# AgentMaker/PAPC

Hardware: AMD Instinct MI355X
Metric: point-clouds/sec (fwd+bwd) PointNet++SSG B=32 N=4096 (higher is better)
Workload: dtype f32

## Files before the change

### papc_amd/csrc/bn_ops.hip

```cpp
#include "common.h"

namespace papc {

template <int V> struct Vec;
template <> struct Vec<4> {
    float4 v;
    __device__ static Vec load(const float *p) { Vec r; r.v = *reinterpret_cast<const float4 *>(p); return r; }
    __device__ void store(float *p) const { *reinterpret_cast<float4 *>(p) = v; }
    __device__ float &operator[](int i) { return (&v.x)[i]; }
    __device__ float operator[](int i) const { return (&v.x)[i]; }
};
template <> struct Vec<1> {
    float v;
    __device__ static Vec load(const float *p) { Vec r; r.v = *p; return r; }
    __device__ void store(float *p) const { *p = v; }
    __device__ float &operator[](int) { return v; }
    __device__ float operator[](int) const { return v; }
};

template <int D>
__device__ __forceinline__ void sum_partial_rows_d(const float *__restrict__ part, int n_tiles, int C, int c, int tl, double &s1, double &s2)
{
    for (int t0 = tl; t0 < n_tiles; t0 += 64 * D) {
        float a[D], b[D];
#pragma unroll
        for (int j = 0; j < D; ++j) {
            const int t = t0 + 64 * j;
            const int64_t o = (int64_t)(t < n_tiles ? t : t0) * 2 * C + c;
            a[j] = part[o];
            b[j] = part[o + C];
        }
#pragma unroll
        for (int j = 0; j < D; ++j) {
            if (t0 + 64 * j < n_tiles) { s1 += (double)a[j]; s2 += (double)b[j]; }
        }
    }
}
__device__ __forceinline__ void sum_partial_rows(const float *__restrict__ part, int n_tiles, int C, int c, int tl, double &s1, double &s2)
{
    if (n_tiles > 512) sum_partial_rows_d<16>(part, n_tiles, C, c, tl, s1, s2);
    else sum_partial_rows_d<8>(part, n_tiles, C, c, tl, s1, s2);
}

__device__ __forceinline__ double lane_get(double v, int l)
{
    const int lo = __builtin_amdgcn_readlane(__double2loint(v), l), hi = __builtin_amdgcn_readlane(__double2hiint(v), l);
    return __hiloint2double(hi, lo);
}
__device__ __forceinline__ void fold_part_lanes(double &s1, double &s2)
{
    s1 += __shfl_xor(s1, 1); s2 += __shfl_xor(s2, 1);
    s1 += __shfl_xor(s1, 2); s2 += __shfl_xor(s2, 2);
    double t1 = 0.0, t2 = 0.0;
#pragma unroll
    for (int w = 0; w < 16; ++w) { t1 += lane_get(s1, 4 * w); t2 += lane_get(s2, 4 * w); }
    s1 = t1; s2 = t2;
}

__device__ __forceinline__ void bn_finalize_channel(const int c, const float *__restrict__ part, int n_tiles, int64_t M, int C,
                                                    const float *__restrict__ gamma, const float *__restrict__ beta,
                                                    float eps, float momentum, float *mean, float *invstd, float *scale,
                                                    float *shift, float *rmean, float *rvar)
{
    const int tl = threadIdx.x;
    const float gam = gamma ? gamma[c] : 1.f, bet = beta ? beta[c] : 0.f;
    const float rm0 = rmean ? rmean[c] : 0.f, rv0 = rvar ? rvar[c] : 0.f;
    double s1 = 0.0, s2 = 0.0;
    sum_partial_rows(part, n_tiles, C, c, tl, s1, s2);
    fold_part_lanes(s1, s2);
    if (tl == 0) {
        const double mu = s1 / (double)M;
        double var = s2 / (double)M - mu * mu;
        if (var < 0.0) var = 0.0;
        const double is = 1.0 / sqrt(var + (double)eps);
        const double sc = (double)gam * is;
        mean[c] = (float)mu;
        invstd[c] = (float)is;
        scale[c] = (float)sc;
        shift[c] = (float)((double)bet - mu * sc);
        if (rmean) rmean[c] = momentum * rm0 + (1.f - momentum) * (float)mu;
        if (rvar) rvar[c] = momentum * rv0 + (1.f - momentum) * (float)var;
    }
}
__global__ __launch_bounds__(64) void bn_finalize_kernel(const float *__restrict__ part, int n_tiles, int64_t M, int C,
                                                        const float *__restrict__ gamma, const float *__restrict__ beta,
                                                        float eps, float momentum, float *mean, float *invstd, float *scale,
                                                        float *shift, float *rmean, float *rvar)
{
    bn_finalize_channel(blockIdx.x, part, n_tiles, M, C, gamma, beta, eps, momentum, mean, invstd, scale, shift, rmean, rvar);
}
constexpr int BN_CLEAR_PER_LANE = 16, BN_CLEAR_PER_WG = 64 * BN_CLEAR_PER_LANE;
__global__ __launch_bounds__(64) void bn_finalize_clear_kernel(const float *__restrict__ part, int n_tiles, int64_t M, int C,
                                                              const float *__restrict__ gamma, const float *__restrict__ beta,
                                                              float eps, float momentum, float *mean, float *invstd, float *scale,
                                                              float *shift, float *rmean, float *rvar, uint4 *__restrict__ clr, int64_t n16)
{
    if ((int)blockIdx.x >= C) {
        const int64_t i0 = (int64_t)((int)blockIdx.x - C) * BN_CLEAR_PER_WG + threadIdx.x;
#pragma unroll
        for (int q = 0; q < BN_CLEAR_PER_LANE; ++q) {
            const int64_t i = i0 + q * 64;
            if (i < n16) clr[i] = make_uint4(0u, 0u, 0u, 0u);
        }
        return;
    }
    bn_finalize_channel(blockIdx.x, part, n_tiles, M, C, gamma, beta, eps, momentum, mean, invstd, scale, shift, rmean, rvar);
}

template <int V>
__global__ __launch_bounds__(256) void bn_relu_max_kernel(const float *__restrict__ y, const float *__restrict__ scale,
                                                          const float *__restrict__ shift, int64_t G, int K, int C,
                                                          float *__restrict__ out, int32_t *__restrict__ argmax)
{
    const int CV = C / V;
    const int64_t total = G * CV;
    for (int64_t e = (int64_t)blockIdx.x * blockDim.x + threadIdx.x; e < total; e += (int64_t)gridDim.x * blockDim.x) {
        const int64_t g = e / CV;
        const int c = (int)(e - g * CV) * V;
        const Vec<V> sc = Vec<V>::load(scale + c), sh = Vec<V>::load(shift + c);
        Vec<V> best;
        int bi[V];
#pragma unroll
        for (int i = 0; i < V; ++i) { best[i] = -1.0f; bi[i] = 0; }
        const float *yp = y + (g * K) * (int64_t)C + c;
        for (int k = 0; k < K; ++k) {
            const Vec<V> v = Vec<V>::load(yp + (int64_t)k * C);
#pragma unroll
            for (int i = 0; i < V; ++i) {
                const float z = relu_np(fmaf(sc[i], v[i], sh[i]));
                if (z > best[i] || z != z) { best[i] = z; bi[i] = k; }
            }
        }
        best.store(out + g * C + c);
        if (argmax) {
#pragma unroll
            for (int i = 0; i < V; ++i) argmax[g * C + c + i] = bi[i];
        }
    }
}

__global__ __launch_bounds__(256) void bn_select_max_kernel(float *__restrict__ gmax, const float *__restrict__ gmin,
                                                            const int32_t *__restrict__ amax, const int32_t *__restrict__ amin,
                                                            const float *__restrict__ scale, const float *__restrict__ shift,
                                                            int64_t total, int C, float *__restrict__ out, int32_t *__restrict__ argmax)
{
    for (int64_t e = (int64_t)blockIdx.x * blockDim.x + threadIdx.x; e < total; e += (int64_t)gridDim.x * blockDim.x) {
        const int c = (int)(e % C);
        const float sc = scale[c], sh = shift[c];
        const bool up = sc >= 0.f;
        const float sel = up ? gmax[e] : gmin[e];
        out[e] = relu_np(fmaf(sc, sel, sh));
        gmax[e] = sel;
        if (argmax) argmax[e] = up ? amax[e] : amin[e];
    }
}

template <int V>
__global__ __launch_bounds__(256) void bn_relu_kernel(const float *__restrict__ y, const float *__restrict__ scale,
                                                      const float *__restrict__ shift, int64_t M, int C, float *__restrict__ z)
{
    const int CV = C / V;
    const int64_t total = M * CV;
    for (int64_t e = (int64_t)blockIdx.x * blockDim.x + threadIdx.x; e < total; e += (int64_t)gridDim.x * blockDim.x) {
        const int c = (int)(e % CV) * V;
        const Vec<V> sc = Vec<V>::load(scale + c), sh = Vec<V>::load(shift + c);
        Vec<V> v = Vec<V>::load(y + e * V);
#pragma unroll
        for (int i = 0; i < V; ++i) v[i] = fmaxf(fmaf(sc[i], v[i], sh[i]), 0.f);
        v.store(z + e * V);
    }
}

template <int V, bool MAXMODE>
__global__ __launch_bounds__(256) void bn_bwd_reduce_kernel(const float *__restrict__ dz, const float *__restrict__ gout,
                                                            const int32_t *__restrict__ argmax, int K,
                                                            const float *__restrict__ y, const float *__restrict__ mean,
                                                            const float *__restrict__ invstd, const float *__restrict__ scale,
                                                            const float *__restrict__ shift, int64_t M, int C,
                                                            float *__restrict__ part, float *__restrict__ psel_out = nullptr)
{
    __shared__ float red[2][256 * 4];
    const int CV = C / V;
    const int CG = CV < 256 ? CV : 256;
    const int RL = 256 / CG;
    const int cgi = threadIdx.x % CG, rl = threadIdx.x / CG;
    const int64_t units = MAXMODE ? M / K : M;
    const int64_t per = (units + gridDim.x - 1) / gridDim.x;
    const int64_t u0 = (int64_t)blockIdx.x * per, u1 = min(units, u0 + per);

    for (int cb = 0; cb < CV; cb += CG) {
        const int cg = cb + cgi;
        Vec<V> a1, a2;
#pragma unroll
        for (int i = 0; i < V; ++i) { a1[i] = 0.f; a2[i] = 0.f; }
        if (cg < CV && rl < RL) {
            const int c = cg * V;
            const Vec<V> sc = Vec<V>::load(scale + c), sh = Vec<V>::load(shift + c);
            const Vec<V> mu = Vec<V>::load(mean + c), is = Vec<V>::load(invstd + c);
            for (int64_t u = u0 + rl; u < u1; u += RL) {
                if (MAXMODE) {
                    Vec<V> g = Vec<V>::load(gout + u * C + c);
                    Vec<V> ys;
                    if (dz) {
                        ys = Vec<V>::load(dz + u * C + c);
                    } else {
#pragma unroll
                        for (int i = 0; i < V; ++i) ys[i] = y[(u * K + argmax[u * C + c + i]) * (int64_t)C + c + i];
                    }
#pragma unroll
                    for (int i = 0; i < V; ++i) {
                        const float yv = ys[i];
                        const float z = fmaf(sc[i], yv, sh[i]);
                        const float p = z > 0.f ? g[i] : 0.f;
                        a1[i] += p;
                        a2[i] = fmaf(p, (yv - mu[i]) * is[i], a2[i]);
                        g[i] = sc[i] * p;
                    }
                    if (psel_out) g.store(psel_out + u * C + c);
                } else {
                    const Vec<V> d = Vec<V>::load(dz + u * C + c);
                    const Vec<V> yv = Vec<V>::load(y + u * C + c);
#pragma unroll
                    for (int i = 0; i < V; ++i) {
                        const float z = fmaf(sc[i], yv[i], sh[i]);
                        const float p = z > 0.f ? d[i] : 0.f;
                        a1[i] += p;
                        a2[i] = fmaf(p, (yv[i] - mu[i]) * is[i], a2[i]);
                    }
                }
            }
        }
#pragma unroll
        for (int i = 0; i < V; ++i) { red[0][threadIdx.x * V + i] = a1[i]; red[1][threadIdx.x * V + i] = a2[i]; }
        __syncthreads();
        for (int t = threadIdx.x; t < CG * V; t += 256) {
            const int c = cb * V + t;
            if (c < C) {
                const int g = t / V, i = t - g * V;
                float s1 = 0.f, s2 = 0.f;
                for (int r = 0; r < RL; ++r) { s1 += red[0][(r * CG + g) * V + i]; s2 += red[1][(r * CG + g) * V + i]; }
                part[((int64_t)blockIdx.x * 2 + 0) * C + c] = s1;
                part[((int64_t)blockIdx.x * 2 + 1) * C + c] = s2;
            }
        }
        __syncthreads();
    }
}

__global__ __launch_bounds__(64) void bn_bwd_finalize_kernel(const float *__restrict__ part, int n_tiles, int64_t M, int C,
                                                            float *dgamma, float *dbeta, float *c1, float *c2, int accumulate)
{
    const int c = blockIdx.x, tl = threadIdx.x;
    double s1 = 0.0, s2 = 0.0;
    sum_partial_rows(part, n_tiles, C, c, tl, s1, s2);
    fold_part_lanes(s1, s2);
    if (tl == 0) {
        if (dbeta) dbeta[c] = (accumulate & 1) ? dbeta[c] + (float)s1 : (float)s1;
        if (dgamma) dgamma[c] = (accumulate & 1) ? dgamma[c] + (float)s2 : (float)s2;
        const bool eval_bn = (accumulate & 2) != 0;
        c1[c] = eval_bn ? 0.f : (float)(s1 / (double)M);
        c2[c] = eval_bn ? 0.f : (float)(s2 / (double)M);
    }
}

__global__ void bn_eval_consts_kernel(const float *__restrict__ rmean, const float *__restrict__ rvar, const float *__restrict__ gamma,
                                      const float *__restrict__ beta, float eps, int C, float *mean, float *invstd, float *scale, float *shift)
{
    const int c = blockIdx.x * blockDim.x + threadIdx.x;
    if (c >= C) return;
    const double mu = (double)rmean[c];
    const double is = 1.0 / sqrt((double)rvar[c] + (double)eps);
    const double sc = (gamma ? (double)gamma[c] : 1.0) * is;
    mean[c] = (float)mu;
    invstd[c] = (float)is;
    scale[c] = (float)sc;
    shift[c] = (float)((beta ? (double)beta[c] : 0.0) - mu * sc);
}

__global__ __launch_bounds__(256) void group_max_bwd_kernel(const float *__restrict__ gout, const int32_t *__restrict__ argmax, int64_t G,
                                                            int K, int C, float *__restrict__ dx)
{
    const int64_t total = G * K * (int64_t)C;
    for (int64_t e = (int64_t)blockIdx.x * blockDim.x + threadIdx.x; e < total; e += (int64_t)gridDim.x * blockDim.x) {
        const int c = (int)(e % C);
        const int64_t m = e / C;
        const int64_t g = m / K;
        const int k = (int)(m - g * K);
        dx[e] = (argmax[g * C + c] == k) ? gout[g * C + c] : 0.f;
    }
}

template <bool ZERO>
__global__ __launch_bounds__(256) void adam_kernel(float *__restrict__ p, float *__restrict__ g, float *__restrict__ m,
                                                   float *__restrict__ v, int64_t n, float lr, float b1, float b2, float omb1, float omb2,
                                                   float eps, float wd, float bc1, float bc2, float gscale)
{
    for (int64_t i = (int64_t)blockIdx.x * blockDim.x + threadIdx.x; i < n; i += (int64_t)gridDim.x * blockDim.x) {
        float gi = g[i] * gscale + wd * p[i];
        const float mi = b1 * m[i] + omb1 * gi;
        const float vi = b2 * v[i] + omb2 * gi * gi;
        m[i] = mi; v[i] = vi;
        p[i] -= lr * (mi / bc1) / (sqrtf(vi / bc2) + eps);
        if (ZERO) g[i] = 0.f;
    }
}

template <bool ZERO, bool TICK, int V>
__global__ __launch_bounds__(256) void adam_dev_kernel(float *__restrict__ p, float *__restrict__ g, float *__restrict__ m,
                                                       float *__restrict__ v, int64_t n, float lr, double beta1, double beta2,
                                                       float eps, float wd, int64_t *__restrict__ step_dev, float gscale)
{
    __shared__ float s_bc[2];
    __shared__ int64_t s_t;
    const int64_t nv = n / V, stride = (int64_t)gridDim.x * blockDim.x, i0 = (int64_t)blockIdx.x * blockDim.x + threadIdx.x;
    Vec<V> gq, pq, mq, vq;
    if (i0 < nv) { gq = Vec<V>::load(g + i0 * V); pq = Vec<V>::load(p + i0 * V); mq = Vec<V>::load(m + i0 * V); vq = Vec<V>::load(v + i0 * V); }
    if (threadIdx.x == 0) {
        const int64_t ti = step_dev[0] + (TICK ? 1 : 0);
        const double t = (double)ti;
        s_t = ti;
        s_bc[0] = (float)(1.0 - pow(beta1, t));
        s_bc[1] = (float)(1.0 - pow(beta2, t));
    }
    __syncthreads();
    const float bc1 = s_bc[0], bc2 = s_bc[1];
    const float b1 = (float)beta1, b2 = (float)beta2, omb1 = (float)(1.0 - beta1), omb2 = (float)(1.0 - beta2);
    for (int64_t i = i0; i < nv; i += stride) {
        if (i != i0) { gq = Vec<V>::load(g + i * V); pq = Vec<V>::load(p + i * V); mq = Vec<V>::load(m + i * V); vq = Vec<V>::load(v + i * V); }
#pragma unroll
        for (int e = 0; e < V; ++e) {
            const float gi = gq[e] * gscale + wd * pq[e];
            const float mi = b1 * mq[e] + omb1 * gi;
            const float vi = b2 * vq[e] + omb2 * gi * gi;
            mq[e] = mi; vq[e] = vi;
            pq[e] -= lr * (mi / bc1) / (sqrtf(vi / bc2) + eps);
            gq[e] = 0.f;
        }
        mq.store(m + i * V); vq.store(v + i * V); pq.store(p + i * V);
        if (ZERO) gq.store(g + i * V);
    }
    if (TICK) {
        __syncthreads();
        if (threadIdx.x == 0) {
            const unsigned long long done = atomicAdd(reinterpret_cast<unsigned long long *>(step_dev + 1), 1ull);
            if (done == (unsigned long long)gridDim.x - 1ull) {
                step_dev[0] = s_t;
                __hip_atomic_store(reinterpret_cast<unsigned long long *>(step_dev + 1), 0ull, __ATOMIC_RELAXED, __HIP_MEMORY_SCOPE_AGENT);
            }
        }
    }
}
__global__ void adam_tick_kernel(int64_t *step_dev) { step_dev[0] += 1; }

__global__ void flag_set_kernel(unsigned *flag, unsigned value, int64_t *counter)
{
    if (counter) counter[0] += 1;
    __hip_atomic_fetch_add(flag, value, __ATOMIC_RELEASE, __HIP_MEMORY_SCOPE_AGENT);
}
__global__ void flag_wait_kernel(unsigned *flag, long long max_spins, int widx)
{
    if (threadIdx.x != 0) return;
    const unsigned want = flag[widx] + 1u;
    long long n = 0;
    while ((int)(__hip_atomic_load(flag, __ATOMIC_ACQUIRE, __HIP_MEMORY_SCOPE_AGENT) - want) < 0) {
        if (n >= max_spins) { __hip_atomic_fetch_add(flag + 2, 1u, __ATOMIC_RELAXED, __HIP_MEMORY_SCOPE_AGENT); break; }
        __builtin_amdgcn_s_sleep(32);
        ++n;
    }
    flag[widx] = want;
}

__global__ __launch_bounds__(256) void fill_kernel(float *__restrict__ p, int64_t n, float v)
{
    const int64_t n4 = n >> 2;
    float4 *p4 = reinterpret_cast<float4 *>(p);
    const float4 v4 = make_float4(v, v, v, v);
    for (int64_t i = (int64_t)blockIdx.x * blockDim.x + threadIdx.x; i < n4; i += (int64_t)gridDim.x * blockDim.x) p4[i] = v4;
    if (blockIdx.x == 0 && threadIdx.x < (n & 3)) p[(n4 << 2) + threadIdx.x] = v;
}

__global__ __launch_bounds__(256) void copy2d_kernel(const float *__restrict__ src, int64_t src_ld, float *__restrict__ dst, int64_t dst_ld,
                                                     int rows, int cols, int transpose)
{
    const int64_t total = (int64_t)rows * cols;
    for (int64_t e = (int64_t)blockIdx.x * blockDim.x + threadIdx.x; e < total; e += (int64_t)gridDim.x * blockDim.x) {
        int r, c;
        if (transpose) { c = (int)(e / rows); r = (int)(e - (int64_t)c * rows); dst[(int64_t)c * dst_ld + r] = src[(int64_t)r * src_ld + c]; }
        else { r = (int)(e / cols); c = (int)(e - (int64_t)r * cols); dst[(int64_t)r * dst_ld + c] = src[(int64_t)r * src_ld + c]; }
    }
}

struct CopyJobs {
    const float *src[8];
    float *dst[8];
    int B[8], R[8], C[8];
    int64_t sb[8], sr[8], sc[8], db[8], dr[8], dc[8];
};

__global__ __launch_bounds__(256) void copy_strided_batch_kernel(CopyJobs j)
{
    __shared__ float tile[32][33];
    const int q = blockIdx.y;
    const int R = j.R[q], C = j.C[q];
    const int tr = (R + 31) >> 5, tc = (C + 31) >> 5;
    const int64_t ntiles = (int64_t)j.B[q] * tr * tc;
    const float *src = j.src[q];
    float *dst = j.dst[q];
    const int64_t sb = j.sb[q], sr = j.sr[q], sc = j.sc[q], db = j.db[q], dr = j.dr[q], dc = j.dc[q];
    const bool src_along_c = sc == 1 || sr != 1, dst_along_c = dc == 1 || dr != 1;
    const int tx = threadIdx.x & 31, ty = threadIdx.x >> 5;
    for (int64_t t = blockIdx.x; t < ntiles; t += gridDim.x) {
        const int b = (int)(t / (tr * tc));
        const int rem = (int)(t - (int64_t)b * tr * tc);
        const int r0 = (rem / tc) * 32, c0 = (rem % tc) * 32;
#pragma unroll
// ... 474 lines not shown
```

### papc_amd/csrc/capi.hip

```cpp
#include <stdarg.h>
#include <string.h>

#include <mutex>
#include <vector>

#include "common.h"

#define GEMM_PARTS_DEFAULT 768

namespace papc {

static thread_local char g_err[512] = "";

void set_error(const char *fmt, ...)
{
    va_list ap;
    va_start(ap, fmt);
    vsnprintf(g_err, sizeof(g_err), fmt, ap);
    va_end(ap);
}

int check_launch(const char *what)
{
    hipError_t e = hipGetLastError();
    if (e != hipSuccess) {
        set_error("%s: %s", what, hipGetErrorString(e));
        return PAPC_E_LAUNCH;
    }
    return PAPC_OK;
}

struct KnobDef { const char *name; int def, lo, hi; };
static const KnobDef g_knob_defs[KNOB_COUNT] = {
    {"PAPC_LG_PARTS", 2048, 1, 8192},
    {"PAPC_DW_F32", 0, 0, 1},
    {"PAPC_DW_DBG", 0, 0, 1},
    {"PAPC_DW_XYZ", 1, 0, 1},
    {"PAPC_PARTS", GEMM_PARTS_DEFAULT, 1, 1024},
    {"PAPC_GEMM_F32", 0, 0, 1},
    {"PAPC_GEMM_WAVES", 0, 0, 8},
    {"PAPC_MAXCAT_WAVES", 8, 4, 8},
    {"PAPC_GEMM_WS", 0, 0, 3},
    {"PAPC_GEMM_OCC", 0, 0, 1},
    {"PAPC_GEMM_DBG", 0, 0, 1},
    {"PAPC_GEMM_KB", 0, 0, 2},
    {"PAPC_GEMM_MINWG", 192, 1, 4096},
    {"PAPC_GEMM_TL", 0, 0, 1},
    {"PAPC_FPS_THREADS", 0, 0, 1024},
    {"PAPC_FPS_THREADS_SMALL", 0, 0, 1024},
    {"PAPC_STREAM", 1, 0, 1},
    {"PAPC_STREAM_MINTILES", 2048, 1, 1 << 30},
    {"PAPC_STREAM_CK", 0, 0, 8},
    {"PAPC_STREAM_ASM", 1, 0, 1},
    {"PAPC_PFN_MFMA", 1, 0, 1},
    {"PAPC_DW_RS64", 1, 0, 1},
    {"PAPC_DW_ROWS", 1, 0, 1},
    {"PAPC_DW_ROWS_BLOCKS", 4, 1, 16},
    {"PAPC_DW_ROWSX", 1, 0, 1},
    {"PAPC_PG_DBG", 0, 0, 15},
    {"PAPC_PG_NB", 0, 0, 2},
    {"PAPC_PG_NS", 0, 0, 3},
    {"PAPC_STREAM_MAXCAT", 1, 0, 1},
    {"PAPC_MAX_NOSTORE", 1, 0, 1},
    {"PAPC_PFN_FUSED_TAILS", 1, 0, 1},
    {"PAPC_STREAM_NW12", 1, 0, 1},
    {"PAPC_LG_LISTS", 1, 0, 1},
    {"PAPC_FOLD_WAVES", 16, 8, 16},
    {"PAPC_LGL_VARIANT", 0, 0, 3},
    {"PAPC_LG_PP", 1, 0, 1},
    {"PAPC_PG_GROUP", 1, 0, 1},
    {"PAPC_PG_PIPE", 1, 0, 1},
    {"PAPC_SEG_EPI", 1, 0, 1},
};
static int g_knobs[KNOB_COUNT];
static int knob_parse(int id, const char *e)
{
    const KnobDef &d = g_knob_defs[id];
    if (!e || !*e) return d.def;
    const int v = atoi(e);
    return (v < d.lo || v > d.hi) ? d.def : v;
}
static const bool g_knobs_loaded = [] {
    for (int i = 0; i < KNOB_COUNT; ++i) g_knobs[i] = knob_parse(i, getenv(g_knob_defs[i].name));
    return true;
}();
int knob(int id) { return g_knobs[id]; }

struct ProfState {
    std::mutex mu;
    unsigned mask = 0;
    std::vector<std::pair<hipEvent_t, hipEvent_t>> pending[PAPC_K_COUNT];
    std::vector<hipEvent_t> pool;
    double total_ms[PAPC_K_COUNT] = {0};
    int64_t launches[PAPC_K_COUNT] = {0};
};
static ProfState g_prof;

static hipEvent_t prof_get_event()
{
    if (!g_prof.pool.empty()) {
        hipEvent_t e = g_prof.pool.back();
        g_prof.pool.pop_back();
        return e;
    }
    hipEvent_t e;
    if (hipEventCreate(&e) != hipSuccess) return nullptr;
    return e;
}

ProfScope::ProfScope(int k, hipStream_t s) : kernel(k), stream(s), on(false), e0(nullptr)
{
    if (!(g_prof.mask & (1u << k))) return;
    std::lock_guard<std::mutex> lk(g_prof.mu);
    e0 = prof_get_event();
    if (!e0) return;
    on = hipEventRecord(e0, stream) == hipSuccess;
}

ProfScope::~ProfScope()
{
    if (!on) return;
    std::lock_guard<std::mutex> lk(g_prof.mu);
    hipEvent_t e1 = prof_get_event();
    if (!e1) return;
    if (hipEventRecord(e1, stream) == hipSuccess) g_prof.pending[kernel].push_back({e0, e1});
}

static void prof_drain(int k)
{
    for (auto &pr : g_prof.pending[k]) {
        float ms = 0.f;
        if (hipEventSynchronize(pr.second) == hipSuccess && hipEventElapsedTime(&ms, pr.first, pr.second) == hipSuccess) {
            g_prof.total_ms[k] += ms;
            g_prof.launches[k] += 1;
        }
        g_prof.pool.push_back(pr.first);
        g_prof.pool.push_back(pr.second);
    }
    g_prof.pending[k].clear();
}

}

extern "C" {

int papc_version(void) { return 600;  }

int papc_abi_version(void) { return PAPC_ABI_VERSION; }

int64_t papc_abi_sizeof(const char *struct_name)
{
    if (!struct_name) return -1;
#define PAPC_SIZEOF(T) if (strcmp(struct_name, #T) == 0) return (int64_t)sizeof(T);
    PAPC_SIZEOF(papc_group_src)
    PAPC_SIZEOF(papc_point_lists)
    PAPC_SIZEOF(papc_group_max)
    PAPC_SIZEOF(papc_bwd_dy)
    PAPC_SIZEOF(papc_scatter_dst)
    PAPC_SIZEOF(papc_bwd_red)
    PAPC_SIZEOF(papc_reduce_job)
    PAPC_SIZEOF(papc_fold_job)
    PAPC_SIZEOF(papc_fold_list)
    PAPC_SIZEOF(papc_sa_desc)
    PAPC_SIZEOF(papc_sa_layer)
    PAPC_SIZEOF(papc_compact_src)
    PAPC_SIZEOF(papc_sa_io)
    PAPC_SIZEOF(papc_sa_plan)
    PAPC_SIZEOF(papc_sa_grads)
    PAPC_SIZEOF(papc_pfn_desc)
    PAPC_SIZEOF(papc_pfn_io)
    PAPC_SIZEOF(papc_det_loss_desc)
    PAPC_SIZEOF(papc_det_loss_io)
    PAPC_SIZEOF(papc_det_post_desc)
    PAPC_SIZEOF(papc_det_post_io)
    PAPC_SIZEOF(papc_head_fc_layer)
    PAPC_SIZEOF(papc_head_bwd_job)
    PAPC_SIZEOF(papc_pg_wjob)
    PAPC_SIZEOF(papc_pg_prep)
    PAPC_SIZEOF(papc_pg_gemm)
    PAPC_SIZEOF(papc_pg_fold_job)
    PAPC_SIZEOF(papc_copy_job)
#undef PAPC_SIZEOF
    return -1;
}

const char *papc_last_error_string(void) { return papc::g_err; }

int papc_knob_set(const char *name, int value)
{
    PAPC_REQUIRE(name, PAPC_E_INVALID, "papc_knob_set: null name");
    for (int i = 0; i < papc::KNOB_COUNT; ++i)
        if (!strcmp(name, papc::g_knob_defs[i].name)) {
            PAPC_REQUIRE(value >= papc::g_knob_defs[i].lo && value <= papc::g_knob_defs[i].hi, PAPC_E_INVALID,
                         "papc_knob_set: %s = %d outside [%d, %d]", name, value, papc::g_knob_defs[i].lo, papc::g_knob_defs[i].hi);
            papc::g_knobs[i] = value;
            return PAPC_OK;
        }
    papc::set_error("papc_knob_set: unknown knob %s", name);
    return PAPC_E_INVALID;
}

int papc_knob_get(const char *name, int *value)
{
    PAPC_REQUIRE(name && value, PAPC_E_INVALID, "papc_knob_get: null argument");
    for (int i = 0; i < papc::KNOB_COUNT; ++i)
        if (!strcmp(name, papc::g_knob_defs[i].name)) { *value = papc::g_knobs[i]; return PAPC_OK; }
    papc::set_error("papc_knob_get: unknown knob %s", name);
    return PAPC_E_INVALID;
}

int papc_prof_enable(unsigned mask)
{
    std::lock_guard<std::mutex> lk(papc::g_prof.mu);
    papc::g_prof.mask = mask;
    return PAPC_OK;
}

int papc_prof_reset(void)
{
    std::lock_guard<std::mutex> lk(papc::g_prof.mu);
    for (int k = 0; k < PAPC_K_COUNT; ++k) {
        papc::prof_drain(k);
        papc::g_prof.total_ms[k] = 0;
        papc::g_prof.launches[k] = 0;
    }
// ... 15 lines not shown
```

### papc_amd/csrc/common.h

```cpp
#pragma once
#include <hip/hip_runtime.h>
#include <stdint.h>
#include <stdio.h>
#include <stdlib.h>
#include <string.h>
#include <algorithm>

#include "papc_hip.h"

namespace papc {

void set_error(const char *fmt, ...);
int check_launch(const char *what);

#define PAPC_REQUIRE(cond, code, ...)      \
    do {                                   \
        if (!(cond)) {                     \
            papc::set_error(__VA_ARGS__);  \
            return (code);                 \
        }                                  \
    } while (0)

enum Knob {
    KNOB_LG_PARTS, KNOB_DW_F32, KNOB_DW_DBG, KNOB_DW_XYZ, KNOB_PARTS, KNOB_GEMM_F32, KNOB_GEMM_WAVES, KNOB_MAXCAT_WAVES,
    KNOB_GEMM_WS, KNOB_GEMM_OCC, KNOB_GEMM_DBG, KNOB_GEMM_KB, KNOB_GEMM_MINWG, KNOB_GEMM_TL, KNOB_FPS_THREADS,
    KNOB_FPS_THREADS_SMALL, KNOB_STREAM, KNOB_STREAM_MINTILES, KNOB_STREAM_CK, KNOB_STREAM_ASM, KNOB_PFN_MFMA, KNOB_DW_RS64, KNOB_DW_ROWS, KNOB_DW_ROWS_BLOCKS, KNOB_DW_ROWSX, KNOB_PG_DBG, KNOB_PG_NB, KNOB_PG_NS, KNOB_STREAM_MAXCAT, KNOB_MAX_NOSTORE, KNOB_PFN_FUSED_TAILS, KNOB_STREAM_NW12, KNOB_LG_LISTS, KNOB_FOLD_WAVES, KNOB_LGL_VARIANT, KNOB_LG_PP, KNOB_PG_GROUP, KNOB_PG_PIPE, KNOB_SEG_EPI, KNOB_COUNT
};
int knob(int id);

struct ProfScope {
    int kernel;
    hipStream_t stream;
    bool on;
    hipEvent_t e0;
    ProfScope(int kernel, hipStream_t stream);
    ~ProfScope();
};

static inline hipStream_t as_stream(papc_stream_t s) { return reinterpret_cast<hipStream_t>(s); }

static inline int64_t cdiv(int64_t a, int64_t b) { return (a + b - 1) / b; }
static inline bool aligned16(const void *p) { return (reinterpret_cast<uintptr_t>(p) & 15) == 0; }

#define PAPC_DPP(v, ctrl, rmask) __builtin_amdgcn_update_dpp((int)(v), (int)(v), (ctrl), (rmask), 0xF, false)

__device__ __forceinline__ float wave_sum_f32_to_lane63(float v)
{
    float t;
    t = __int_as_float(PAPC_DPP(__float_as_int(v), 0xB1, 0xF));  v += t;
    t = __int_as_float(PAPC_DPP(__float_as_int(v), 0x4E, 0xF));  v += t;
    t = __int_as_float(PAPC_DPP(__float_as_int(v), 0x124, 0xF)); v += t;
    t = __int_as_float(PAPC_DPP(__float_as_int(v), 0x128, 0xF)); v += t;
    t = __int_as_float(__builtin_amdgcn_update_dpp(0, __float_as_int(v), 0x142, 0xA, 0xF, false)); v += t;
    t = __int_as_float(__builtin_amdgcn_update_dpp(0, __float_as_int(v), 0x143, 0xC, 0xF, false)); v += t;
    return v;
}

__device__ __forceinline__ float half_sum_f32(float v)
{
    float t;
    t = __int_as_float(PAPC_DPP(__float_as_int(v), 0xB1, 0xF));  v += t;
    t = __int_as_float(PAPC_DPP(__float_as_int(v), 0x4E, 0xF));  v += t;
    t = __int_as_float(PAPC_DPP(__float_as_int(v), 0x124, 0xF)); v += t;
    t = __int_as_float(PAPC_DPP(__float_as_int(v), 0x128, 0xF)); v += t;
    t = __int_as_float(__builtin_amdgcn_update_dpp(0, __float_as_int(v), 0x142, 0xA, 0xF, false)); v += t;
    return v;
}

__device__ __forceinline__ float readlane63_f32(float v)
{
    return __int_as_float(__builtin_amdgcn_readlane(__float_as_int(v), 63));
}


#define PAPC_DPPF(v, ctrl, rmask) __int_as_float(__builtin_amdgcn_update_dpp(__float_as_int(v), __float_as_int(v), (ctrl), (rmask), 0xF, false))
#define PAPC_DPPU(v, ctrl, rmask) ((unsigned)__builtin_amdgcn_update_dpp((int)(v), (int)(v), (ctrl), (rmask), 0xF, false))

__device__ __forceinline__ float row_max_f32(float v)
{
    v = fmaxf(v, PAPC_DPPF(v, 0xB1, 0xF));
    v = fmaxf(v, PAPC_DPPF(v, 0x4E, 0xF));
    v = fmaxf(v, PAPC_DPPF(v, 0x124, 0xF));
    v = fmaxf(v, PAPC_DPPF(v, 0x128, 0xF));
    return v;
}
__device__ __forceinline__ unsigned row_min_u32(unsigned v)
{
    unsigned t;
    t = PAPC_DPPU(v, 0xB1, 0xF);  v = t < v ? t : v;
    t = PAPC_DPPU(v, 0x4E, 0xF);  v = t < v ? t : v;
    t = PAPC_DPPU(v, 0x124, 0xF); v = t < v ? t : v;
    t = PAPC_DPPU(v, 0x128, 0xF); v = t < v ? t : v;
    return v;
}
__device__ __forceinline__ float wave_max_f32_to_lane63(float v)
{
    v = row_max_f32(v);
    v = fmaxf(v, PAPC_DPPF(v, 0x142, 0xA));
    v = fmaxf(v, PAPC_DPPF(v, 0x143, 0xC));
    return v;
}
__device__ __forceinline__ unsigned wave_min_u32_to_lane63(unsigned v)
{
    unsigned t;
    v = row_min_u32(v);
    t = PAPC_DPPU(v, 0x142, 0xA); v = t < v ? t : v;
    t = PAPC_DPPU(v, 0x143, 0xC); v = t < v ? t : v;
    return v;
}
#define PAPC_DPP_STEP(op, v, ctrl) asm volatile("s_nop 1\n\t" op " %0, %0, %0 " ctrl : "+v"(v))
__device__ __forceinline__ unsigned row_max_u32_fused(unsigned v)
{
    PAPC_DPP_STEP("v_max_u32_dpp", v, "quad_perm:[1,0,3,2] row_mask:0xf bank_mask:0xf");
    PAPC_DPP_STEP("v_max_u32_dpp", v, "quad_perm:[2,3,0,1] row_mask:0xf bank_mask:0xf");
    PAPC_DPP_STEP("v_max_u32_dpp", v, "row_ror:4 row_mask:0xf bank_mask:0xf");
    PAPC_DPP_STEP("v_max_u32_dpp", v, "row_ror:8 row_mask:0xf bank_mask:0xf");
    return v;
}
__device__ __forceinline__ unsigned row_min_u32_fused(unsigned v)
{
    PAPC_DPP_STEP("v_min_u32_dpp", v, "quad_perm:[1,0,3,2] row_mask:0xf bank_mask:0xf");
    PAPC_DPP_STEP("v_min_u32_dpp", v, "quad_perm:[2,3,0,1] row_mask:0xf bank_mask:0xf");
    PAPC_DPP_STEP("v_min_u32_dpp", v, "row_ror:4 row_mask:0xf bank_mask:0xf");
    PAPC_DPP_STEP("v_min_u32_dpp", v, "row_ror:8 row_mask:0xf bank_mask:0xf");
    return v;
}
__device__ __forceinline__ unsigned wave_max_u32_fused_to_lane63(unsigned v)
{
    v = row_max_u32_fused(v);
    PAPC_DPP_STEP("v_max_u32_dpp", v, "row_bcast:15 row_mask:0xa bank_mask:0xf");
    PAPC_DPP_STEP("v_max_u32_dpp", v, "row_bcast:31 row_mask:0xc bank_mask:0xf");
    asm volatile("s_nop 1" ::"v"(v));
    return v;
}
__device__ __forceinline__ unsigned wave_min_u32_fused_to_lane63(unsigned v)
{
    v = row_min_u32_fused(v);
    PAPC_DPP_STEP("v_min_u32_dpp", v, "row_bcast:15 row_mask:0xa bank_mask:0xf");
    PAPC_DPP_STEP("v_min_u32_dpp", v, "row_bcast:31 row_mask:0xc bank_mask:0xf");
    asm volatile("s_nop 1" ::"v"(v));
    return v;
}
__device__ __forceinline__ unsigned readlane63_u32(unsigned v) { return (unsigned)__builtin_amdgcn_readlane((int)v, 63); }
__device__ __forceinline__ float readlane0_f32(float v) { return __int_as_float(__builtin_amdgcn_readlane(__float_as_int(v), 0)); }
__device__ __forceinline__ unsigned readlane0_u32(unsigned v) { return (unsigned)__builtin_amdgcn_readlane((int)v, 0); }

__device__ __forceinline__ void lds_barrier()
{
    asm volatile("s_waitcnt lgkmcnt(0)\n\ts_barrier" ::: "memory");
}

__device__ __forceinline__ float relu_np(float t) { return !(t <= 0.f) ? t : 0.f; }
__device__ __forceinline__ int lane_id() { return (int)(threadIdx.x & 63); }

}
```

### papc_amd/csrc/mlp_dw.hip

```cpp
#include <type_traits>
#include "mlp_loaders.h"

namespace papc {

template <int I, int N, class F>
__device__ __forceinline__ void dw_sfor(F &&f)
{
    if constexpr (I < N) {
        f(std::integral_constant<int, I>{});
        dw_sfor<I + 1, N>(f);
    }
}

void fill_dy(DySrc &d, const papc_bwd_dy *s);
int check_dy(const papc_bwd_dy *dy, int64_t M, int C, bool *vec, const char *who);
int fill_asrc(ASrc &a, int a_mode, const float *x, int64_t ldx, const papc_group_src *grp, const float *sc,
              const float *sh, int Cin, const char *who);

struct DwArgs {
    ASrc x;
    ASrc dy;
    int64_t M; int Cin; int Cout; int rows_per_chunk;
    float *dw_partial;
    float *db_partial;
    int64_t part_ld;
    int xmap;
    int TOp, TIp;
    int RS;
    unsigned long long *dbg;
};

constexpr int DW_T = 128;
constexpr int DW_TI_WIDE = 160;
constexpr int DW_STAGE_FLOATS = 9216;

template <int XMODE, int DYMODE, bool VEC, int WO, int WI, int NTO, int NTI, int NSX>
__global__ __launch_bounds__(256, 2) void dw_kernel(DwArgs p)
{
    static_assert(WO * WI == 4, "4 waves");
    __shared__ __attribute__((aligned(16))) float smem[2 * DW_STAGE_FLOATS + DW_T];
    float *dbred = smem + 2 * DW_STAGE_FLOATS;

    const int tid = threadIdx.x, lane = tid & 63, wave = tid >> 6;
    const int hi = lane >> 5, l31 = lane & 31;
    const int wo = wave / WI, wi = wave % WI;
    const int o0 = blockIdx.y * DW_T, i0 = blockIdx.z * (NSX > 4 ? DW_TI_WIDE : DW_T);
    const int TOp = p.TOp, TIp = p.TIp, RS = p.RS;
    const int nto = min(TOp / 32, (p.Cout - o0 + 31) / 32);
    const int nti = min(TIp / 32, (p.Cin - i0 + 31) / 32);
    const int cgy = TOp / 4, cgx = TIp / 4;
    const int nsy = (RS * cgy + 255) / 256, nsx = (RS * cgx + 255) / 256;
    int yr[4], xr[NSX], xk[NSX];
    const int kqy = (tid % cgy) * 4;
#pragma unroll
    for (int i = 0; i < 4; ++i) yr[i] = (tid + 256 * (i < nsy ? i : nsy - 1)) / cgy;
#pragma unroll
    for (int i = 0; i < NSX; ++i) {
        const int s = tid + 256 * (i < nsx ? i : nsx - 1);
        xr[i] = s / cgx;
        xk[i] = (s - xr[i] * cgx) * 4;
    }
    const int kqx = xk[0];
    const bool use_jpre = (XMODE == A_GROUP) && p.x.g.idx != nullptr;

    floatx16 acc[NTO][NTI];
#pragma unroll
    for (int a = 0; a < NTO; ++a)
#pragma unroll
        for (int b = 0; b < NTI; ++b)
#pragma unroll
            for (int r = 0; r < 16; ++r) acc[a][b][r] = 0.f;
    int toff[NTO], tiff[NTI];
    bool tok_o[NTO], tok_i[NTI];
#pragma unroll
    for (int a = 0; a < NTO; ++a) { const int to = wo * NTO + a; tok_o[a] = to < nto; toff[a] = (tok_o[a] ? to : 0) * 32; }
#pragma unroll
    for (int b = 0; b < NTI; ++b) { const int ti = wi * NTI + b; tok_i[b] = ti < nti; tiff[b] = (tok_i[b] ? ti : 0) * 32; }

    const KConst kcy = make_kconst<DYMODE, VEC>(p.dy, o0 + kqy, p.Cout);
    const KConst kcx = make_kconst<XMODE, VEC>(p.x, i0 + kqx, p.Cin);
    float4 dbs = make_float4(0.f, 0.f, 0.f, 0.f);

    const int64_t mbeg = (int64_t)blockIdx.x * p.rows_per_chunk;
    const int64_t mend = min(p.M, mbeg + p.rows_per_chunk);

    RowCtx rowy[4], rowx[NSX];
    Raw3 rawy[4], rawx[NSX];
    int jpre[NSX];
#pragma unroll
    for (int i = 0; i < NSX; ++i) jpre[i] = -2;

    auto prefetch_j = [&](int64_t m0) {
        if (use_jpre) {
#pragma unroll
            for (int i = 0; i < NSX; ++i) {
                const int64_t m = m0 + xr[i];
                jpre[i] = p.x.g.idx[m < p.M ? m : 0];
            }
        }
    };
    auto fetch = [&](int64_t m0) {
#pragma unroll
        for (int i = 0; i < 4; ++i) {
            rowy[i] = make_row<DYMODE>(p.dy, m0 + yr[i], mend);
            rawy[i] = fetch_a4<DYMODE, VEC>(p.dy, rowy[i], o0 + kqy, p.Cout);
        }
#pragma unroll
        for (int i = 0; i < NSX; ++i) {
            rowx[i] = make_row<XMODE>(p.x, m0 + xr[i], mend, use_jpre ? jpre[i] : -2);
            rawx[i] = fetch_a4<XMODE, VEC>(p.x, rowx[i], i0 + xk[i], p.Cin);
        }
    };
    auto finish = [&](float *Ys, float *Xs) {
#pragma unroll
        for (int i = 0; i < 4; ++i) {
            const float4 vy = finish_a4<DYMODE, VEC>(p.dy, rowy[i], o0 + kqy, p.Cout, kcy, rawy[i]);
            if (i < nsy) { dbs.x += vy.x; dbs.y += vy.y; dbs.z += vy.z; dbs.w += vy.w; }
            *reinterpret_cast<float4 *>(&Ys[yr[i] * TOp + kqy]) = vy;
        }
#pragma unroll
        for (int i = 0; i < NSX; ++i) {
            const float4 vx = finish_a4<XMODE, VEC>(p.x, rowx[i], i0 + xk[i], p.Cin, kcx, rawx[i]);
            *reinterpret_cast<float4 *>(&Xs[xr[i] * TIp + xk[i]]) = vx;
        }
    };

    bool have = mbeg < mend;
    if (have) {
        prefetch_j(mbeg);
        fetch(mbeg);
        prefetch_j(mbeg + RS);
        finish(smem, smem + RS * TOp);
    }
    __syncthreads();
    int buf = 0;
    int64_t m0 = mbeg;
    while (have) {
        const int64_t mn = m0 + RS;
        const bool have_next = mn < mend;
        if (have_next) {
            fetch(mn);
            prefetch_j(mn + RS);
        }
        {
            const float *Ys = smem + buf * DW_STAGE_FLOATS + hi * TOp + l31;
            const float *Xs = smem + buf * DW_STAGE_FLOATS + RS * TOp + hi * TIp + l31;
            const int nks = RS / 2;
            float a0[NTO], b0[NTI], a1[NTO], b1[NTI];
#pragma unroll
            for (int a = 0; a < NTO; ++a) a0[a] = Ys[toff[a]];
#pragma unroll
            for (int b = 0; b < NTI; ++b) b0[b] = Xs[tiff[b]];
            for (int ks = 0; ks < nks; ks += 2) {
                const float *y1 = Ys + (2 * ks + 2) * TOp, *x1 = Xs + (2 * ks + 2) * TIp;
#pragma unroll
                for (int a = 0; a < NTO; ++a) a1[a] = y1[toff[a]];
#pragma unroll
                for (int b = 0; b < NTI; ++b) b1[b] = x1[tiff[b]];
#pragma unroll
                for (int a = 0; a < NTO; ++a)
#pragma unroll
                    for (int b = 0; b < NTI; ++b) acc[a][b] = __builtin_amdgcn_mfma_f32_32x32x2f32(a0[a], b0[b], acc[a][b], 0, 0, 0);
                const int k2 = (ks + 2 < nks) ? ks + 2 : ks;
                const float *y2 = Ys + (2 * k2) * TOp, *x2 = Xs + (2 * k2) * TIp;
#pragma unroll
                for (int a = 0; a < NTO; ++a) a0[a] = y2[toff[a]];
#pragma unroll
                for (int b = 0; b < NTI; ++b) b0[b] = x2[tiff[b]];
#pragma unroll
                for (int a = 0; a < NTO; ++a)
#pragma unroll
                    for (int b = 0; b < NTI; ++b) acc[a][b] = __builtin_amdgcn_mfma_f32_32x32x2f32(a1[a], b1[b], acc[a][b], 0, 0, 0);
            }
        }
        if (have_next) {
            float *Ys = smem + (buf ^ 1) * DW_STAGE_FLOATS;
            finish(Ys, Ys + RS * TOp);
        }
        lds_barrier();
        buf ^= 1;
        m0 = mn;
        have = have_next;
// ... 360 lines not shown
    for (int a = 0; a < NTO; ++a) {
        const int c = o0 + 32 * a + l31;
        ksc[a] = d.scale[c]; ksh[a] = d.shift[c]; kmu[a] = d.mean[c];
        kA[a] = ksc[a] * d.c1[c];
        kB[a] = ksc[a] * d.c2[c] * d.invstd[c];
    }
#pragma unroll
    for (int b = 0; b < NTI; ++b) {
        if (XYZ) { xs[b] = 0.f; xh[b] = 0.f; }
        else { xs[b] = p.x.sc[i0 + 32 * b + l31]; xh[b] = p.x.sh[i0 + 32 * b + l31]; }
    }
    float4 wfk[NTI];
#pragma unroll
    for (int b = 0; b < NTI; ++b) wfk[b] = XYZ ? ld4(p.x.sc + 4 * (i0 + 32 * b + l31)) : make_float4(0.f, 0.f, 0.f, 0.f);

    floatx16 acc[NTO][NTI];
#pragma unroll
    for (int a = 0; a < NTO; ++a)
#pragma unroll
        for (int b = 0; b < NTI; ++b)
#pragma unroll
            for (int r = 0; r < 16; ++r) acc[a][b][r] = 0.f;

    struct Raw { float y[NTO][8], z[NTO][8], x[XYZ ? 3 : NTI][8]; int am[NTO]; };
    auto ldg = [](const float *base, uint32_t byte_off) { return *reinterpret_cast<const float *>(reinterpret_cast<const char *>(base) + byte_off); };
    auto ldgi = [](const int *base, uint32_t byte_off) { return *reinterpret_cast<const int *>(reinterpret_cast<const char *>(base) + byte_off); };
    const uint32_t ystride = (uint32_t)Cout * 4u, xstride = (uint32_t)(XYZ ? 4 : ldx) * 4u;
    const uint32_t oy_lane = (uint32_t)((mbeg + 8 * hi) * Cout + o0 + l31) * 4u;
    const uint32_t ox_lane = XYZ ? (uint32_t)((mbeg + 8 * hi) * 4) * 4u : (uint32_t)((mbeg + 8 * hi) * ldx + i0 + l31) * 4u;
    auto fetch = [&](int kb, Raw &w) {
        const uint32_t oy = oy_lane + (uint32_t)kb * 16u * ystride, ox = ox_lane + (uint32_t)kb * 16u * xstride;
#pragma unroll
        for (int j = 0; j < 8; ++j) {
#pragma unroll
            for (int a = 0; a < NTO; ++a) {
                w.y[a][j] = ldg(d.y, oy + (uint32_t)j * ystride + 128u * a);
                if (DYMODE == A_DY_DENSE) w.z[a][j] = ldg(d.dz, oy + (uint32_t)j * ystride + 128u * a);
            }
            if (XYZ) {
                w.x[0][j] = ldg(p.x.x, ox + (uint32_t)j * 16u); w.x[1][j] = ldg(p.x.x, ox + (uint32_t)j * 16u + 4u); w.x[2][j] = ldg(p.x.x, ox + (uint32_t)j * 16u + 8u);
            } else {
#pragma unroll
                for (int b = 0; b < NTI; ++b) w.x[b][j] = ldg(p.x.x, ox + (uint32_t)j * xstride + 128u * b);
            }
        }
        if (DYMODE == A_DY_MAX) {
            const uint32_t g = fdiv((uint32_t)mbeg + 16u * (uint32_t)kb, d.divK);
            const uint32_t og = (g * (uint32_t)Cout + (uint32_t)(o0 + l31)) * 4u;
#pragma unroll
            for (int a = 0; a < NTO; ++a) {
                w.z[a][0] = ldg(d.gout, og + 128u * a);
                w.am[a] = ldgi(d.argmax, og + 128u * a);
            }
        }
    };
    auto compute = [&](int kb, const Raw &w) {
        int kin0 = 0;
        if (DYMODE == A_DY_MAX) {
            const uint32_t b0 = (uint32_t)mbeg + 16u * (uint32_t)kb;
            kin0 = (int)(b0 - fdiv(b0, d.divK) * (uint32_t)d.K) + 8 * hi;
        }
        bf16x8 pa[NTO][3], pb[NTI][3];
#pragma unroll
        for (int a = 0; a < NTO; ++a) {
            float v[8];
#pragma unroll
            for (int j = 0; j < 8; ++j) {
                const float y = w.y[a][j];
                float dz;
                if (DYMODE == A_DY_DENSE) dz = w.z[a][j];
                else dz = (w.am[a] == kin0 + j) ? w.z[a][0] : 0.f;
                const float z = fmaf(ksc[a], y, ksh[a]);
                const float pp = z > 0.f ? dz : 0.f;
                v[j] = fmaf(ksc[a], pp, -fmaf(kB[a], y - kmu[a], kA[a]));
            }
            split8(v, pa[a]);
        }
#pragma unroll
        for (int b = 0; b < NTI; ++b) {
            float v[8];
#pragma unroll
            for (int j = 0; j < 8; ++j) {
                if (XYZ) v[j] = fmaxf(fmaf(wfk[b].z, w.x[2][j], fmaf(wfk[b].y, w.x[1][j], fmaf(wfk[b].x, w.x[0][j], wfk[b].w))), 0.f);
                else v[j] = fmaxf(fmaf(xs[b], w.x[b][j], xh[b]), 0.f);
            }
            split8(v, pb[b]);
        }
#pragma unroll
        for (int t = 0; t < 6; ++t)
#pragma unroll
            for (int a = 0; a < NTO; ++a)
#pragma unroll
                for (int b = 0; b < NTI; ++b)
                    acc[a][b] = __builtin_amdgcn_mfma_f32_32x32x16_bf16(pa[a][BF16X3_PA[t]], pb[b][BF16X3_PB[t]], acc[a][b], 0, 0, 0);
    };

    constexpr int PF = (DYMODE == A_DY_MAX && !XYZ) ? 3 : 2;
    const int nb = (n_kb - wave + 7) >> 3;
    if (nb > 0) {
        const int last = wave + 8 * (nb - 1);
        Raw rr[PF];
#pragma unroll
        for (int i = 0; i < PF - 1; ++i) fetch(min(wave + 8 * i, last), rr[i]);
        const int n_main = nb - nb % PF;
        for (int j0 = 0; j0 < n_main; j0 += PF) {
#pragma unroll
            for (int i = 0; i < PF; ++i) {
                const int kb = wave + 8 * (j0 + i);
                fetch(min(kb + 8 * (PF - 1), last), rr[(i + PF - 1) % PF]);
                __builtin_amdgcn_sched_barrier(0);
                compute(kb, rr[i]);
                __builtin_amdgcn_sched_barrier(0);
            }
        }
#pragma unroll
        for (int i = 0; i < PF - 1; ++i)
            if (n_main + i < nb) compute(wave + 8 * (n_main + i), rr[i]);
    }

#pragma unroll
    for (int half = 4; half >= 1; half >>= 1) {
        if (wave >= half && wave < 2 * half) {
#pragma unroll
            for (int a = 0; a < NTO; ++a)
#pragma unroll
                for (int b = 0; b < NTI; ++b)
#pragma unroll
                    for (int r = 0; r < 16; ++r) slab[wave - half][(a * NTI + b) * 16 + r][lane] = acc[a][b][r];
        }
        __syncthreads();
        if (wave < half) {
#pragma unroll
            for (int a = 0; a < NTO; ++a)
#pragma unroll
                for (int b = 0; b < NTI; ++b)
#pragma unroll
                    for (int r = 0; r < 16; ++r) acc[a][b][r] += slab[wave][(a * NTI + b) * 16 + r][lane];
        }
        __syncthreads();
    }
    if (wave == 0) {
        float *out = p.dw_partial + (int64_t)blockIdx.x * p.part_ld;
#pragma unroll
        for (int a = 0; a < NTO; ++a)
#pragma unroll
            for (int b = 0; b < NTI; ++b)
#pragma unroll
                for (int r = 0; r < 16; ++r) {
                    const int co = o0 + 32 * a + (r & 3) + 8 * (r >> 2) + 4 * hi;
                    out[(int64_t)co * p.Cin + i0 + 32 * b + l31] = acc[a][b][r];
                }
    }
    if (p.db_partial && blockIdx.z == 0 && tid < 64) p.db_partial[(int64_t)blockIdx.x * p.part_ld + o0 + tid] = 0.f;
}

template <int DYMODE, int NW, bool CP = false, bool RG = false>
__global__ __launch_bounds__(64 * NW, 2) void dw_rowsx_kernel(DwArgs p)
{
    static_assert(!(CP && RG), "ragged widths: padded stacks only");
    constexpr int NTI = 4, CI = 128, CHS = 48, PLB = CI * CHS, STG = 3 * PLB;
    constexpr int CB = 32 * NW;
    constexpr int RPT = 32 / NW;
    constexpr int NX4 = RPT / 4;
    __shared__ __attribute__((aligned(16))) char xs_lds[2 * STG];
    const int tid = threadIdx.x, lane = tid & 63, wave = tid >> 6;
    const int hi = lane >> 5, l31 = lane & 31;
    const int co = RG ? min((int)blockIdx.y * CB + wave * 32 + l31, p.Cout - 1) : blockIdx.y * CB + wave * 32 + l31;
    const DySrc &d = p.dy.d;
    const int i0 = RG ? (int)blockIdx.z * CI : 0;
    const uint32_t LDX = RG ? (uint32_t)p.x.ldx : (uint32_t)CI;
    int64_t rows_all = p.M, rpc = p.rows_per_chunk;
    if constexpr (CP) {
        rows_all = __builtin_amdgcn_readfirstlane(*d.rows_dev);
        rpc = (((rows_all + gridDim.x - 1) / gridDim.x) + 15) & ~(int64_t)15;
    }
    const int64_t mbeg = (int64_t)blockIdx.x * rpc;
    const int64_t mend = min(rows_all, mbeg + rpc);
    const int n_kb = mbeg < mend ? (int)((mend - mbeg) >> 4) : 0;
    const int Cout = p.Cout;

    const float ksc = d.scale[co], ksh = d.shift[co], kmu = d.mean[co];
    const float kA = ksc * d.c1[co], kB = ksc * d.c2[co] * d.invstd[co];
    const int xc = tid & 127, xq = tid >> 7;
    const int xg = RG ? min(i0 + xc, p.Cin - 1) : xc;
    const float xsc = p.x.sc[xg], xsh = p.x.sh[xg];

    floatx16 acc[NTI];
#pragma unroll
    for (int b = 0; b < NTI; ++b)
#pragma unroll
        for (int r = 0; r < 16; ++r) acc[b][r] = 0.f;

    struct Raw { float y[8], z[8]; int am; float4 w0, w1; int g; };
    struct RawX { float x[RPT]; };
    auto ldg = [](const float *base, uint32_t byte_off) { return *reinterpret_cast<const float *>(reinterpret_cast<const char *>(base) + byte_off); };
    auto ldgi = [](const int *base, uint32_t byte_off) { return *reinterpret_cast<const int *>(reinterpret_cast<const char *>(base) + byte_off); };
    const uint32_t ystride = (uint32_t)Cout * 4u;
    const uint32_t oy_lane = (uint32_t)((mbeg + 8 * hi) * Cout + co) * 4u;
    const uint32_t ox_lane = (uint32_t)((mbeg + RPT * xq) * LDX + xg) * 4u;
    const uint32_t ow_lane = (uint32_t)(mbeg + 8 * hi) * 4u;
    const uint32_t og_lane = (uint32_t)(((mbeg >> 3) + hi)) * 4u;
    auto fetch_g = [&](int kb, Raw &w) {
        if constexpr (CP && DYMODE == A_DY_MAX) w.g = ldgi(d.seg_grp, og_lane + (uint32_t)kb * 8u);
    };
    auto fetch = [&](int kb, Raw &w) {
        const uint32_t o0 = oy_lane + (uint32_t)kb * 16u * ystride;
#pragma unroll
        for (int j = 0; j < 8; ++j) {
            w.y[j] = ldg(d.y, o0 + (uint32_t)j * ystride);
            if (DYMODE == A_DY_DENSE) w.z[j] = ldg(d.dz, o0 + (uint32_t)j * ystride);
        }
        if (DYMODE == A_DY_MAX) {
            uint32_t g;
            if constexpr (CP) g = (uint32_t)w.g;
            else g = fdiv((uint32_t)mbeg + 16u * (uint32_t)kb, d.divK);
            const uint32_t og = (g * (uint32_t)Cout + (uint32_t)co) * 4u;
            w.z[0] = ldg(d.gout, og);
            w.am = ldgi(d.argmax, og);
        }
        if constexpr (CP) {
            const char *wb = reinterpret_cast<const char *>(d.wrow) + ow_lane + (uint32_t)kb * 64u;
            w.w0 = *reinterpret_cast<const float4 *>(wb);
            w.w1 = *reinterpret_cast<const float4 *>(wb + 16);
        }
    };
    auto wof = [](const Raw &w, int j) -> float {
        const float a[8] = {w.w0.x, w.w0.y, w.w0.z, w.w0.w, w.w1.x, w.w1.y, w.w1.z, w.w1.w};
        return a[j];
    };
    auto fetch_x = [&](int kb, RawX &w) {
        const uint32_t o0 = ox_lane + (uint32_t)kb * (16u * LDX * 4u);
#pragma unroll
        for (int j = 0; j < RPT; ++j) w.x[j] = ldg(p.x.x, o0 + (uint32_t)j * (LDX * 4u));
    };
    auto stage_x = [&](int kb, const RawX &w, char *stg) {
        (void)kb;
#pragma unroll
        for (int h = 0; h < NX4; ++h) {
            float4 v;
            v.x = fmaxf(fmaf(xsc, w.x[4 * h + 0], xsh), 0.f); v.y = fmaxf(fmaf(xsc, w.x[4 * h + 1], xsh), 0.f);
            v.z = fmaxf(fmaf(xsc, w.x[4 * h + 2], xsh), 0.f); v.w = fmaxf(fmaf(xsc, w.x[4 * h + 3], xsh), 0.f);
            uint2 q0, q1, q2;
            split3(v, q0, q1, q2);
            char *dst = stg + xc * CHS + xq * (2 * RPT) + 8 * h;
            *reinterpret_cast<uint2 *>(dst) = q0;
            *reinterpret_cast<uint2 *>(dst + PLB) = q1;
            *reinterpret_cast<uint2 *>(dst + 2 * PLB) = q2;
        }
    };
    auto prep = [&](int kb, const Raw &w, bf16x8 (&pa)[3]) {
        int kin0 = 0;
        if (DYMODE == A_DY_MAX) {
            const uint32_t b0 = (uint32_t)mbeg + 16u * (uint32_t)kb;
            kin0 = CP ? (int)b0 + 8 * hi : (int)(b0 - fdiv(b0, d.divK) * (uint32_t)d.K) + 8 * hi;
        }
        float v[8];
#pragma unroll
        for (int j = 0; j < 8; ++j) {
            const float y = w.y[j];
            float dz;
            if (DYMODE == A_DY_DENSE) dz = w.z[j];
            else dz = (w.am == kin0 + j) ? w.z[0] : 0.f;
            const float z = fmaf(ksc, y, ksh);
            const float pp = z > 0.f ? dz : 0.f;
            if constexpr (CP) v[j] = fmaf(-wof(w, j), fmaf(kB, y - kmu, kA), ksc * pp);
            else v[j] = fmaf(ksc, pp, -fmaf(kB, y - kmu, kA));
        }
        split8(v, pa);
    };
    auto mma = [&](const bf16x8 (&pa)[3], const char *stg) {
        bf16x8 pb[NTI][3];
#pragma unroll
        for (int b = 0; b < NTI; ++b)
#pragma unroll
            for (int pl = 0; pl < 3; ++pl)
                pb[b][pl] = *reinterpret_cast<const bf16x8 *>(stg + pl * PLB + (32 * b + l31) * CHS + hi * 16);
#pragma unroll
        for (int t = 0; t < 6; ++t)
#pragma unroll
            for (int b = 0; b < NTI; ++b)
                acc[b] = __builtin_amdgcn_mfma_f32_32x32x16_bf16(pa[BF16X3_PA[t]], pb[b][BF16X3_PB[t]], acc[b], 0, 0, 0);
    };

    auto weave = [&](const bf16x8 (&pc)[3], const char *stg, int kbn, const Raw &w, bf16x8 (&pn)[3], const RawX &wx, char *stgn) {
        bf16x8 pb[NTI][3];
#pragma unroll
        for (int pl = 0; pl < 3; ++pl)
#pragma unroll
            for (int b = 0; b < NTI; ++b)
                pb[b][pl] = *reinterpret_cast<const bf16x8 *>(stg + pl * PLB + (32 * b + l31) * CHS + hi * 16);
        int kin0 = 0;
        if (DYMODE == A_DY_MAX) {
            const uint32_t b0 = (uint32_t)mbeg + 16u * (uint32_t)kbn;
            kin0 = CP ? (int)b0 + 8 * hi : (int)(b0 - fdiv(b0, d.divK) * (uint32_t)d.K) + 8 * hi;
        }
        float v[8];
        float4 ra, rb, rx;
        uint2 a0, a1, a2, b0, b1, b2, q0, q1, q2;
        auto pin = [](float &x) { asm volatile("" : "+v"(x)); };
        auto pin4 = [&](float4 &r) { pin(r.x); pin(r.y); pin(r.z); pin(r.w); };
        auto pinu = [](uint2 &u) { asm volatile("" : "+v"(u.x), "+v"(u.y)); };
        dw_sfor<0, 24>([&](auto g_) {
            constexpr int g = decltype(g_)::value, t = g / NTI, bb = g % NTI;
            acc[bb] = __builtin_amdgcn_mfma_f32_32x32x16_bf16(pc[BF16X3_PA[t]], pb[bb][BF16X3_PB[t]], acc[bb], 0, 0, 0);
            __builtin_amdgcn_sched_barrier(0);
            if constexpr (g < 8) {
                const float y = w.y[g];
                float dz;
                if (DYMODE == A_DY_DENSE) dz = w.z[g];
                else dz = (w.am == kin0 + g) ? w.z[0] : 0.f;
                const float z = fmaf(ksc, y, ksh);
                const float pp = z > 0.f ? dz : 0.f;
                if constexpr (CP) v[g] = fmaf(-wof(w, g), fmaf(kB, y - kmu, kA), ksc * pp);
                else v[g] = fmaf(ksc, pp, -fmaf(kB, y - kmu, kA));
                pin(v[g]);
            } else if constexpr (g == 8) { ra = make_float4(v[0], v[1], v[2], v[3]); split_level(ra, a0); pin4(ra); pinu(a0); }
            else if constexpr (g == 9) { split_level(ra, a1); pin4(ra); pinu(a1); }
            else if constexpr (g == 10) {
                a2.x = pack_bf16x2(ra.x, ra.y); a2.y = pack_bf16x2(ra.z, ra.w); rb = make_float4(v[4], v[5], v[6], v[7]); split_level(rb, b0);
                pinu(a2); pin4(rb); pinu(b0);
            } else if constexpr (g == 11) { split_level(rb, b1); pin4(rb); pinu(b1); }
            else if constexpr (g == 12) {
                b2.x = pack_bf16x2(rb.x, rb.y); b2.y = pack_bf16x2(rb.z, rb.w);
                pinu(b2);
                pn[0] = __builtin_bit_cast(bf16x8, make_uint4(a0.x, a0.y, b0.x, b0.y));
                pn[1] = __builtin_bit_cast(bf16x8, make_uint4(a1.x, a1.y, b1.x, b1.y));
                pn[2] = __builtin_bit_cast(bf16x8, make_uint4(a2.x, a2.y, b2.x, b2.y));
            } else if constexpr (g >= 13 && g < 13 + 4 * NX4) {
                constexpr int h = (g - 13) / 4, step = (g - 13) % 4;
                if constexpr (step == 0) {
                    rx.x = fmaxf(fmaf(xsc, wx.x[4 * h + 0], xsh), 0.f); rx.y = fmaxf(fmaf(xsc, wx.x[4 * h + 1], xsh), 0.f);
                    rx.z = fmaxf(fmaf(xsc, wx.x[4 * h + 2], xsh), 0.f); rx.w = fmaxf(fmaf(xsc, wx.x[4 * h + 3], xsh), 0.f);
                    pin4(rx);
                } else if constexpr (step == 1) { split_level(rx, q0); pin4(rx); pinu(q0); }
                else if constexpr (step == 2) { split_level(rx, q1); pin4(rx); pinu(q1); }
                else {
                    q2.x = pack_bf16x2(rx.x, rx.y); q2.y = pack_bf16x2(rx.z, rx.w);
                    char *dst = stgn + xc * CHS + xq * (2 * RPT) + 8 * h;
                    *reinterpret_cast<uint2 *>(dst) = q0;
                    *reinterpret_cast<uint2 *>(dst + PLB) = q1;
                    *reinterpret_cast<uint2 *>(dst + 2 * PLB) = q2;
                }
            }
            __builtin_amdgcn_sched_barrier(0);
        });
    };

    constexpr int PF = 3;
    Raw dr[PF];
    RawX xr[PF];
    bf16x8 pa[PF][3];
    const int last = n_kb - 1;
    if (n_kb > 0) {
#pragma unroll
        for (int i = 0; i < PF; ++i) fetch_g(min(i, last), dr[i]);
#pragma unroll
        for (int i = 0; i < PF - 1; ++i) { fetch(min(i, last), dr[i]); fetch_x(min(i, last), xr[i]); }
        stage_x(0, xr[0], xs_lds);
        prep(0, dr[0], pa[0]);
        lds_barrier();
    }
    const int n_main = n_kb - n_kb % PF;
    for (int kb0 = 0; kb0 < n_main; kb0 += PF) {
#pragma unroll
        for (int i = 0; i < PF; ++i) {
            const int kb = kb0 + i;
            constexpr int NXT = PF - 1;
            if constexpr (CP && DYMODE == A_DY_MAX) {
                const int gnew = ldgi(d.seg_grp, og_lane + (uint32_t)min(kb + PF, last) * 8u);
                fetch(min(kb + NXT, last), dr[(i + NXT) % PF]);
                dr[i].g = gnew;
            } else
            fetch(min(kb + NXT, last), dr[(i + NXT) % PF]);
            fetch_x(min(kb + NXT, last), xr[(i + NXT) % PF]);
            __builtin_amdgcn_sched_barrier(0);
            weave(pa[i], xs_lds + (kb & 1) * STG, min(kb + 1, last), dr[(i + 1) % PF], pa[(i + 1) % PF], xr[(i + 1) % PF],
                  xs_lds + ((kb + 1) & 1) * STG);
            lds_barrier();
        }
    }
#pragma unroll
    for (int i = 0; i < PF - 1; ++i) {
        const int kb = n_main + i;
        if (kb < n_kb) {
            mma(pa[i], xs_lds + (kb & 1) * STG);
            if (kb + 1 < n_kb) {
                prep(kb + 1, dr[(i + 1) % PF], pa[(i + 1) % PF]);
                stage_x(kb + 1, xr[(i + 1) % PF], xs_lds + ((kb + 1) & 1) * STG);
            }
            lds_barrier();
        }
    }

    float *out = p.dw_partial + (int64_t)blockIdx.x * p.part_ld;
    const int cbase = blockIdx.y * CB + wave * 32;
#pragma unroll
    for (int b = 0; b < NTI; ++b)
#pragma unroll
        for (int r = 0; r < 16; ++r) {
            const int c = cbase + (r & 3) + 8 * (r >> 2) + 4 * hi;
            if constexpr (RG) {
                if (c < p.Cout && i0 + 32 * b + l31 < p.Cin) out[(int64_t)c * p.Cin + i0 + 32 * b + l31] = acc[b][r];
            } else
            out[(int64_t)c * CI + 32 * b + l31] = acc[b][r];
        }
    if (p.db_partial && tid < CB && (!RG || (blockIdx.z == 0 && (int)blockIdx.y * CB + tid < p.Cout))) p.db_partial[(int64_t)blockIdx.x * p.part_ld + blockIdx.y * CB + tid] = 0.f;
}

static unsigned long long *g_dw_dbg = nullptr;
struct DwMaxArgs {
    const float *x, *xsc, *xsh, *psel;
    const int *argmax;
    float *partial;
    int64_t M, part_ld;
    int K, Cout, rows_per_chunk, n_chunks;
};

__global__ __launch_bounds__(512, 2) void dw_rows_max_kernel(DwMaxArgs p)
{
    constexpr int NT = 3, NTI = 2, CI = 64;
    __shared__ float slab[4][NT * NTI * 16][64];
    const int tid = threadIdx.x, lane = tid & 63, wave = tid >> 6;
    const int hi = lane >> 5, l31 = lane & 31;
    const int yb = (blockIdx.x >> 3) & 1, chunk = (int)(((blockIdx.x >> 4) << 3) | (blockIdx.x & 7));
    const int o0 = 64 * yb, Cout = p.Cout;
    const int64_t mbeg = (int64_t)chunk * p.rows_per_chunk;
    const int64_t mend = min(p.M, mbeg + p.rows_per_chunk);
    const int n_kb = mbeg < mend ? (int)((mend - mbeg) >> 4) : 0;
    const int kshift = 31 - __clz(p.K);

    float xs[NTI], xh[NTI], xsum[NTI];
#pragma unroll
    for (int b = 0; b < NTI; ++b) { xs[b] = p.xsc[32 * b + l31]; xh[b] = p.xsh[32 * b + l31]; xsum[b] = 0.f; }
    floatx16 acc[NT][NTI];
#pragma unroll
    for (int a = 0; a < NT; ++a)
#pragma unroll
        for (int b = 0; b < NTI; ++b)
#pragma unroll
            for (int r = 0; r < 16; ++r) acc[a][b][r] = 0.f;

    struct Raw { float x[NTI][8]; float ps[2]; int am[2]; };
    auto ldg = [](const float *base, uint32_t byte_off) { return *reinterpret_cast<const float *>(reinterpret_cast<const char *>(base) + byte_off); };
    auto ldgi = [](const int *base, uint32_t byte_off) { return *reinterpret_cast<const int *>(reinterpret_cast<const char *>(base) + byte_off); };
    const uint32_t ox_lane = (uint32_t)((mbeg + 8 * hi) * CI + l31) * 4u;
    const uint32_t og_lane = (uint32_t)(o0 + l31) * 4u;
    auto fetch = [&](int kb, Raw &w) {
        const uint32_t o = ox_lane + (uint32_t)kb * (16u * CI * 4u);
#pragma unroll
        for (int j = 0; j < 8; ++j)
#pragma unroll
            for (int b = 0; b < NTI; ++b) w.x[b][j] = ldg(p.x, o + (uint32_t)(j * CI + 32 * b) * 4u);
        const uint32_t g = ((uint32_t)mbeg + 16u * (uint32_t)kb) >> kshift;
        const uint32_t og = g * (uint32_t)Cout * 4u + og_lane;
#pragma unroll
        for (int a = 0; a < 2; ++a) {
            w.ps[a] = ldg(p.psel, og + 128u * a);
            w.am[a] = ldgi(p.argmax, og + 128u * a);
        }
    };
    auto compute = [&](int kb, const Raw &w) {
        const int kin0 = (int)(((uint32_t)mbeg + 16u * (uint32_t)kb) & (uint32_t)(p.K - 1)) + 8 * hi;
        bf16x8 pa[2][3], pb[NTI][3];
#pragma unroll
        for (int b = 0; b < NTI; ++b) {
            float v[8];
#pragma unroll
            for (int j = 0; j < 8; ++j) { v[j] = fmaxf(fmaf(xs[b], w.x[b][j], xh[b]), 0.f); xsum[b] += v[j]; }
            split8(v, pb[b]);
        }
        {
            uint2 q0, q1, q2;
            split3(make_float4(w.ps[0], w.ps[1], 0.f, 0.f), q0, q1, q2);
            const unsigned pl[3] = {q0.x, q1.x, q2.x};
#pragma unroll
            for (int a = 0; a < 2; ++a) {
                const int idx = w.am[a] - kin0;
                const int dsel = (idx >= 0 && idx < 8) ? (idx >> 1) : -1;
                const int sh = (idx & 1) * 16;
#pragma unroll
                for (int t = 0; t < 3; ++t) {
                    const unsigned bits = ((a ? pl[t] >> 16 : pl[t]) & 0xffffu) << sh;
                    pa[a][t] = __builtin_bit_cast(bf16x8, make_uint4(dsel == 0 ? bits : 0u, dsel == 1 ? bits : 0u, dsel == 2 ? bits : 0u, dsel == 3 ? bits : 0u));
                }
            }
        }
        bf16x8 pg[3];
#pragma unroll
        for (int t = 0; t < 3; ++t) pg[t] = yb ? pb[1][t] : pb[0][t];
#pragma unroll
        for (int t = 0; t < 6; ++t)
#pragma unroll
            for (int b = 0; b < NTI; ++b) {
                acc[0][b] = __builtin_amdgcn_mfma_f32_32x32x16_bf16(pa[0][BF16X3_PA[t]], pb[b][BF16X3_PB[t]], acc[0][b], 0, 0, 0);
                acc[1][b] = __builtin_amdgcn_mfma_f32_32x32x16_bf16(pa[1][BF16X3_PA[t]], pb[b][BF16X3_PB[t]], acc[1][b], 0, 0, 0);
                acc[2][b] = __builtin_amdgcn_mfma_f32_32x32x16_bf16(pg[BF16X3_PA[t]], pb[b][BF16X3_PB[t]], acc[2][b], 0, 0, 0);
            }
    };

    constexpr int PF = 3;
    const int nb = (n_kb - wave + 7) >> 3;
    if (nb > 0) {
        const int last = wave + 8 * (nb - 1);
        Raw rr[PF];
#pragma unroll
        for (int i = 0; i < PF - 1; ++i) fetch(min(wave + 8 * i, last), rr[i]);
        const int n_main = nb - nb % PF;
        for (int j0 = 0; j0 < n_main; j0 += PF) {
#pragma unroll
            for (int i = 0; i < PF; ++i) {
                const int kb = wave + 8 * (j0 + i);
                fetch(min(kb + 8 * (PF - 1), last), rr[(i + PF - 1) % PF]);
                __builtin_amdgcn_sched_barrier(0);
                compute(kb, rr[i]);
                __builtin_amdgcn_sched_barrier(0);
            }
        }
#pragma unroll
        for (int i = 0; i < PF - 1; ++i)
            if (n_main + i < nb) compute(wave + 8 * (n_main + i), rr[i]);
    }

    float *out = p.partial + (int64_t)chunk * p.part_ld;
    if (yb == 0) {
        float *sred = &slab[0][0][0];
#pragma unroll
        for (int b = 0; b < NTI; ++b) sred[(wave * 2 + hi) * CI + 32 * b + l31] = xsum[b];
        __syncthreads();
        if (tid < CI) {
            float sacc = 0.f;
            for (int q = 0; q < 16; ++q) sacc += sred[q * CI + tid];
            out[(int64_t)(Cout + CI) * CI + tid] = sacc;
        }
        __syncthreads();
    }
#pragma unroll
    for (int half = 4; half >= 1; half >>= 1) {
        if (wave >= half && wave < 2 * half) {
#pragma unroll
            for (int a = 0; a < NT; ++a)
#pragma unroll
                for (int b = 0; b < NTI; ++b)
#pragma unroll
                    for (int r = 0; r < 16; ++r) slab[wave - half][(a * NTI + b) * 16 + r][lane] = acc[a][b][r];
        }
        __syncthreads();
        if (wave < half) {
#pragma unroll
            for (int a = 0; a < NT; ++a)
#pragma unroll
                for (int b = 0; b < NTI; ++b)
#pragma unroll
                    for (int r = 0; r < 16; ++r) acc[a][b][r] += slab[wave][(a * NTI + b) * 16 + r][lane];
        }
        __syncthreads();
    }
    if (wave == 0) {
#pragma unroll
        for (int a = 0; a < NT; ++a)
#pragma unroll
            for (int b = 0; b < NTI; ++b)
#pragma unroll
                for (int r = 0; r < 16; ++r) {
                    const int rr = (r & 3) + 8 * (r >> 2) + 4 * hi;
                    const int row = a < 2 ? o0 + 32 * a + rr : Cout + 32 * yb + rr;
                    out[(int64_t)row * CI + 32 * b + l31] = acc[a][b][r];
                }
    }
}

__global__ __launch_bounds__(64) void dw_max_fold_kernel(const float *__restrict__ partial, int n_chunks, int64_t part_ld, int n, double *__restrict__ out)
{
    const int l = threadIdx.x & 15, q = threadIdx.x >> 4;
    const int e = blockIdx.x * 16 + l;
    const int per = (n_chunks + 3) / 4, c0 = q * per, c1 = min(n_chunks, c0 + per);
    double s = 0.0;
    if (e < n) {
        int c = c0;
        for (; c + 8 <= c1; c += 8) {
            float v[8];
#pragma unroll
            for (int j = 0; j < 8; ++j) v[j] = partial[(int64_t)(c + j) * part_ld + e];
#pragma unroll
            for (int j = 0; j < 8; ++j) s += (double)v[j];
        }
        for (; c < c1; ++c) s += (double)partial[(int64_t)c * part_ld + e];
    }
    const double s1 = __shfl(s, l + 16), s2 = __shfl(s, l + 32), s3 = __shfl(s, l + 48);
    if (q == 0 && e < n) out[e] = ((s + s1) + s2) + s3;
}

__global__ __launch_bounds__(256) void dw_max_finalize_kernel(const double *__restrict__ fold, const float *__restrict__ w, const float *__restrict__ e,
                                                              const float *__restrict__ scale, const float *__restrict__ c1, double inv_m, int Cout,
                                                              float *__restrict__ dw, int accumulate)
{
    constexpr int CI = 64;
    __shared__ double gc[CI][CI];
    const int tid = threadIdx.x;
    const double *G = fold + (int64_t)Cout * CI, *S = G + CI * CI;
    for (int q = tid; q < CI * CI; q += 256) {
        const int j = q >> 6, i = q & 63;
        gc[j][i] = G[q] - S[j] * S[i] * inv_m;
    }
    __syncthreads();
    const int i = tid & 63, c = 4 * blockIdx.x + (tid >> 6);
    if (c >= Cout) return;
    double dot = 0.0;
    for (int j = 0; j < CI; ++j) dot += (double)w[(int64_t)c * CI + j] * gc[j][i];
    const double v = fold[(int64_t)c * CI + i] - (double)scale[c] * (double)c1[c] * S[i] - (double)e[c] * dot;
    float *o = dw + (int64_t)c * CI + i;
    *o = accumulate ? *o + (float)v : (float)v;
}

static void dw_dbg_report(const DwArgs &p, int xm, int dm)
{
    hipDeviceSynchronize();
    unsigned long long h[32];
    hipMemcpy(h, g_dw_dbg, sizeof(h), hipMemcpyDeviceToHost);
    const double n = (double)h[4];
    fprintf(stderr, "[dw dbg] x %d dy %d M %lld Cout %d Cin %d: slots %.0f | consumer cyc/slot: reads+mfma-issue %.0f barrier %.0f | producer grp0 per ACTIVE slot: wait %.0f finish %.0f issue %.0f ; barrier/slot %.0f\n",
            xm, dm, (long long)p.M, p.Cout, p.Cin, n, h[0] / n, h[1] / n, h[8] / n, h[9] / n, h[10] / n, h[11] / n);
}

static bool dw_rowsx_ragged(int Cin, int Cout)
{
    return (Cin == 128 && Cout == 196) || (Cin == 196 && Cout == 256) || (Cin == 96 && Cout == 128) || (Cin == 64 && Cout == 96);
}
static bool dw_rowsx_eligible(int Cin, int Cout, bool dense, int K)
{
    return knob(KNOB_DW_ROWSX) != 0 && ((Cin == 128 && Cout % 128 == 0) || dw_rowsx_ragged(Cin, Cout)) && !dw_f32_exact() && (dense || (K >= 16 && K % 16 == 0));
}
static bool dw_rows_eligible(int Cin, int Cout, bool dense, int K)
{
    return knob(KNOB_DW_ROWS) != 0 && Cin % 64 == 0 && Cout % 64 == 0 && (Cin / 64) * (Cout / 64) <= knob(KNOB_DW_ROWS_BLOCKS) && !dw_f32_exact() && (dense || (K >= 16 && K % 16 == 0));
}

template <int XMODE, int DYMODE, bool VEC>
static int launch_dw_v(const DwArgs &p_in, hipStream_t st)
{
    DwArgs p = p_in;
    const int dbg_on = knob(KNOB_DW_DBG);
    if (dbg_on) {
        if (!g_dw_dbg) hipMalloc(&g_dw_dbg, 32 * sizeof(unsigned long long));
        hipMemsetAsync(g_dw_dbg, 0, 32 * sizeof(unsigned long long), st);
        p.dbg = g_dw_dbg;
    }
    const bool wide = p.TIp == DW_TI_WIDE;
    dim3 grid((unsigned)cdiv(p.M, p.rows_per_chunk), (unsigned)cdiv(p.Cout, DW_T), (unsigned)cdiv(p.Cin, wide ? DW_TI_WIDE : DW_T));
    const int to = p.TOp / 32, ti = p.TIp / 32;
    const bool off32 = (int64_t)p.rows_per_chunk * std::max<int64_t>(p.Cout, XMODE == A_GROUP ? 1 : p.x.ldx) * 4 < (1ll << 31);
    const bool k4 = DYMODE != A_DY_MAX || p.dy.d.K % 4 == 0;
    const bool rowsx_rows_ok = p.M % 16 == 0 && p.M * (int64_t)p.Cout * 4 < (1ll << 32);
    if (p.dy.d.wrow) {
        const bool ok = VEC && XMODE == A_BNRELU && rowsx_rows_ok && p.Cin == 128 && p.Cout % 128 == 0 && p.x.ldx == p.Cin && !dw_f32_exact() &&
                        p.dy.d.rows_dev && (DYMODE != A_DY_MAX || p.dy.d.seg_grp) && p.M % 128 == 0;
        if (!ok) {
            set_error("papc_mlp_bwd_dw_f32: a compacted dY source needs a 128-channel BN+ReLU input and Cout %% 128 == 0 (got Cin=%d Cout=%d)", p.Cin, p.Cout);
            return PAPC_E_UNSUPPORTED;
        }
        if (p.Cout % 256 == 0) {
            dim3 g2((unsigned)cdiv(p.M, p.rows_per_chunk), (unsigned)(p.Cout / 256));
            hipLaunchKernelGGL((dw_rowsx_kernel<DYMODE, 8, true>), g2, dim3(512), 0, st, p);
        } else {
            dim3 g2((unsigned)cdiv(p.M, p.rows_per_chunk), (unsigned)(p.Cout / 128));
            hipLaunchKernelGGL((dw_rowsx_kernel<DYMODE, 4, true>), g2, dim3(256), 0, st, p);
        }
        return check_launch("papc_mlp_bwd_dw_f32 (compacted)");
    }
    if (VEC && XMODE == A_BNRELU && rowsx_rows_ok && dw_rowsx_eligible(p.Cin, p.Cout, DYMODE == A_DY_DENSE, p.dy.d.K) && p.x.ldx == p.Cin && p.rows_per_chunk % 16 == 0 &&
        (!dw_rowsx_ragged(p.Cin, p.Cout) || p.M * (int64_t)p.Cin * 4 < (1ll << 32))) {
        if (dw_rowsx_ragged(p.Cin, p.Cout) && p.Cout <= 128) {
            dim3 g2((unsigned)cdiv(p.M, p.rows_per_chunk), 1u, (unsigned)cdiv(p.Cin, 128));
            hipLaunchKernelGGL((dw_rowsx_kernel<DYMODE, 4, false, true>), g2, dim3(256), 0, st, p);
        } else if (dw_rowsx_ragged(p.Cin, p.Cout)) {
            dim3 g2((unsigned)cdiv(p.M, p.rows_per_chunk), (unsigned)cdiv(p.Cout, 256), (unsigned)cdiv(p.Cin, 128));
            hipLaunchKernelGGL((dw_rowsx_kernel<DYMODE, 8, false, true>), g2, dim3(512), 0, st, p);
        } else if (p.Cout % 256 == 0) {
            dim3 g2((unsigned)cdiv(p.M, p.rows_per_chunk), (unsigned)(p.Cout / 256));
            hipLaunchKernelGGL((dw_rowsx_kernel<DYMODE, 8>), g2, dim3(512), 0, st, p);
        } else {
            dim3 g2((unsigned)cdiv(p.M, p.rows_per_chunk), (unsigned)(p.Cout / 128));
            hipLaunchKernelGGL((dw_rowsx_kernel<DYMODE, 4>), g2, dim3(256), 0, st, p);
        }
        return check_launch("papc_mlp_bwd_dw_f32");
    }
    const bool rows_rows_ok = p.M % 16 == 0 && p.M * (int64_t)std::max(p.Cout, p.Cin) * 4 < (1ll << 32);
    if (VEC && XMODE == A_BNRELU && rows_rows_ok && dw_rows_eligible(p.Cin, p.Cout, DYMODE == A_DY_DENSE, p.dy.d.K) && p.x.ldx == p.Cin && p.rows_per_chunk % 16 == 0) {
        dim3 g2((unsigned)cdiv(p.M, p.rows_per_chunk), (unsigned)(p.Cout / 64), (unsigned)(p.Cin / 64));
        hipLaunchKernelGGL((dw_rows_kernel<DYMODE>), g2, dim3(512), 0, st, p);
        return check_launch("papc_mlp_bwd_dw_f32");
    }
    if (VEC && XMODE != A_GROUP && !wide && to >= 2 && ti >= 2 && off32 && k4 && !dw_f32_exact()) {
        if (to > 2 && ti > 2) hipLaunchKernelGGL((dw_ws_kernel<XMODE, DYMODE, 2, 2>), grid, dim3(768), 0, st, p);
        else if (to > 2) hipLaunchKernelGGL((dw_ws_kernel<XMODE, DYMODE, 2, 1>), grid, dim3(768), 0, st, p);
        else if (ti > 2) hipLaunchKernelGGL((dw_ws_kernel<XMODE, DYMODE, 1, 2>), grid, dim3(768), 0, st, p);
        else if (knob(KNOB_DW_RS64)) hipLaunchKernelGGL((dw_ws_kernel<XMODE, DYMODE, 1, 1, 64>), grid, dim3(768), 0, st, p);
        else hipLaunchKernelGGL((dw_ws_kernel<XMODE, DYMODE, 1, 1>), grid, dim3(768), 0, st, p);
        if (dbg_on) dw_dbg_report(p, XMODE, DYMODE);
        return check_launch("papc_mlp_bwd_dw_f32");
    }
    if (wide) {
        if (XMODE == A_GROUP) hipLaunchKernelGGL((dw_kernel<A_GROUP, DYMODE, VEC, 4, 1, 1, 5, 5>), grid, dim3(256), 0, st, p);
    } else if (!VEC) {
        hipLaunchKernelGGL((dw_kernel<XMODE, DYMODE, false, 2, 2, 2, 2, 4>), grid, dim3(256), 0, st, p);
    } else if (to > 2 && ti > 2) hipLaunchKernelGGL((dw_kernel<XMODE, DYMODE, VEC, 2, 2, 2, 2, 4>), grid, dim3(256), 0, st, p);
    else if (to > 2) hipLaunchKernelGGL((dw_kernel<XMODE, DYMODE, VEC, 2, 2, 2, 1, 4>), grid, dim3(256), 0, st, p);
    else if (ti > 2) hipLaunchKernelGGL((dw_kernel<XMODE, DYMODE, VEC, 2, 2, 1, 2, 4>), grid, dim3(256), 0, st, p);
    else hipLaunchKernelGGL((dw_kernel<XMODE, DYMODE, VEC, 2, 2, 1, 1, 4>), grid, dim3(256), 0, st, p);
    return check_launch("papc_mlp_bwd_dw_f32");
}

template <int XMODE, int DYMODE>
static int launch_dw(const DwArgs &p, bool vec, hipStream_t st)
{
    return vec ? launch_dw_v<XMODE, DYMODE, true>(p, st) : launch_dw_v<XMODE, DYMODE, false>(p, st);
}

static int pad_tile(int c) { return c <= 32 ? 32 : (c <= 64 ? 64 : 128); }

}

using namespace papc;

extern "C" int papc_mlp_bwd_dw_chunk_hint(int64_t M, int Cin, int Cout, int a_mode, int dz_mode, int K)
{
    if (a_mode == PAPC_A_GROUP && dz_mode == PAPC_DZ_DENSE && (Cin == 3 || Cin == 7) && knob(KNOB_DW_XYZ) && Cout % 4 == 0 && Cout <= 256 && M >= 1) {
        const int64_t rpc = std::max<int64_t>(256, cdiv(cdiv(M, 2048), 64) * 64);
        return (int)std::min<int64_t>(rpc, 1 << 24);
    }
    if ((a_mode != PAPC_A_BNRELU && a_mode != PAPC_A_XYZ) || M < 1) return 0;
    const bool xk = dw_rowsx_eligible(Cin, Cout, dz_mode == PAPC_DZ_DENSE, K);
    if (!xk && !dw_rows_eligible(Cin, Cout, dz_mode == PAPC_DZ_DENSE, K)) return 0;
    hipDeviceProp_t prop;
    int dev = 0;
    static int ncu = 0;
    if (!ncu) { ncu = 256; if (hipGetDevice(&dev) == hipSuccess && hipGetDeviceProperties(&prop, dev) == hipSuccess && prop.multiProcessorCount > 0) ncu = prop.multiProcessorCount; }
    const int64_t want = xk ? (dw_rowsx_ragged(Cin, Cout) ? std::max<int64_t>(1, (Cout <= 128 ? 2 : 1) * ncu / (cdiv(Cout, 256) * cdiv(Cin, 128)))
                                  : Cout % 256 == 0 ? std::max<int64_t>(1, ncu / (Cout / 256)) : std::max<int64_t>(1, 2 * ncu / (Cout / 128)))
                            : std::max<int64_t>(1, ncu / ((Cout / 64) * (Cin / 64)));
    int64_t rpc = cdiv(M, want);
    rpc = std::max<int64_t>(64, cdiv(rpc, 64) * 64);
    return (int)std::min<int64_t>(rpc, 1 << 24);
}

extern "C" int papc_mlp_bwd_dw_f32(const papc_bwd_dy *dy, int a_mode, const float *x, int64_t ldx,
                                   const papc_group_src *grp, const float *bn_scale, const float *bn_shift, int64_t M,
                                   int Cin, int Cout, int rows_per_chunk, float *dw_partial, float *db_partial,
                                   int64_t part_ld, papc_stream_t stream)
{
    PAPC_REQUIRE(dw_partial, PAPC_E_INVALID, "papc_mlp_bwd_dw_f32: null dw_partial");
    PAPC_REQUIRE(M >= 1 && Cin >= 1 && Cout >= 1, PAPC_E_INVALID, "papc_mlp_bwd_dw_f32: bad sizes");
    PAPC_REQUIRE(M < (1ll << 31), PAPC_E_UNSUPPORTED, "papc_mlp_bwd_dw_f32: M=%lld >= 2^31 rows", (long long)M);
    PAPC_REQUIRE(part_ld >= (int64_t)Cout * Cin, PAPC_E_INVALID, "papc_mlp_bwd_dw_f32: part_ld=%lld < Cout*Cin", (long long)part_ld);
    PAPC_REQUIRE(rows_per_chunk >= 64 && rows_per_chunk % 64 == 0, PAPC_E_INVALID,
                 "papc_mlp_bwd_dw_f32: rows_per_chunk=%d must be a positive multiple of 64", rows_per_chunk);
    bool vdy = false;
    int rc = check_dy(dy, M, Cout, &vdy, "papc_mlp_bwd_dw_f32");
    if (rc) return rc;
    DwArgs p;
    memset(&p, 0, sizeof(p));
    rc = fill_asrc(p.x, a_mode, x, ldx, grp, bn_scale, bn_shift, Cin, "papc_mlp_bwd_dw_f32");
    if (rc) return rc;
    if (a_mode == A_XYZ) {
        const bool dense_ = dy->dz_mode == PAPC_DZ_DENSE;
        PAPC_REQUIRE(vdy && p.x.vec && dw_rows_eligible(Cin, Cout, dense_, dy->K) && rows_per_chunk % 16 == 0 && M % 16 == 0 &&
                     M * (int64_t)Cout * 4 < (1ll << 32), PAPC_E_UNSUPPORTED,
                     "papc_mlp_bwd_dw_f32: PAPC_A_XYZ is not built for Cin=%d Cout=%d (see papc_mlp_xyz_ok)", Cin, Cout);
        fill_dy(p.dy.d, dy);
        p.dy.d.C = Cout;
        p.M = M; p.Cin = Cin; p.Cout = Cout; p.rows_per_chunk = rows_per_chunk; p.dw_partial = dw_partial; p.db_partial = db_partial; p.part_ld = part_ld;
        hipStream_t st2 = as_stream(stream);
        ProfScope prof2(PAPC_K_BWD_DW, st2);
        dim3 g2((unsigned)cdiv(M, rows_per_chunk), (unsigned)(Cout / 64), (unsigned)(Cin / 64));
        if (dense_) hipLaunchKernelGGL((dw_rows_kernel<A_DY_DENSE, true>), g2, dim3(512), 0, st2, p);
        else hipLaunchKernelGGL((dw_rows_kernel<A_DY_MAX, true>), g2, dim3(512), 0, st2, p);
        return check_launch("papc_mlp_bwd_dw_f32");
    }
    fill_dy(p.dy.d, dy);
    p.dy.d.C = Cout;
    const bool vec = vdy && p.x.vec;
    p.M = M; p.Cin = Cin; p.Cout = Cout; p.rows_per_chunk = rows_per_chunk; p.dw_partial = dw_partial; p.db_partial = db_partial; p.part_ld = part_ld;
    p.xmap = (a_mode == A_GROUP) ? 1 : 0;
    p.TOp = pad_tile(Cout); p.TIp = pad_tile(Cin);
    if (a_mode == A_GROUP && Cin > DW_T && Cin <= DW_TI_WIDE && p.TOp == 128) p.TIp = DW_TI_WIDE;
    p.RS = (p.TOp + p.TIp <= 128) ? 64 : 32;
    hipStream_t st = as_stream(stream);
    ProfScope prof(PAPC_K_BWD_DW, st);
    const bool dense = dy->dz_mode == PAPC_DZ_DENSE;
    const int xyz_on = knob(KNOB_DW_XYZ);
    if (xyz_on && a_mode == A_GROUP && dense && vec && ((grp->D == 0 && Cin == 3) || (grp->D == 4 && Cin == 7)) && Cout % 4 == 0 && Cout >= 4 && Cout <= 256) {
        if (grp->D == 0) hipLaunchKernelGGL(dw_xyz_kernel<0>, dim3((unsigned)cdiv(M, rows_per_chunk)), dim3(256), 0, st, p);
        else hipLaunchKernelGGL(dw_xyz_kernel<1>, dim3((unsigned)cdiv(M, rows_per_chunk)), dim3(256), 0, st, p);
        return check_launch("papc_mlp_bwd_dw_f32");
    }
    switch (a_mode) {
    case A_PLAIN: return dense ? launch_dw<A_PLAIN, A_DY_DENSE>(p, vec, st) : launch_dw<A_PLAIN, A_DY_MAX>(p, vec, st);
    case A_BNRELU: return dense ? launch_dw<A_BNRELU, A_DY_DENSE>(p, vec, st) : launch_dw<A_BNRELU, A_DY_MAX>(p, vec, st);
    default: return dense ? launch_dw<A_GROUP, A_DY_DENSE>(p, vec, st) : launch_dw<A_GROUP, A_DY_MAX>(p, vec, st);
    }
}

static int dw_max_chunks()
{
    static int n = 0;
    if (!n) {
        hipDeviceProp_t prop;
        int dev = 0, ncu = 256;
        if (hipGetDevice(&dev) == hipSuccess && hipGetDeviceProperties(&prop, dev) == hipSuccess && prop.multiProcessorCount > 0) ncu = prop.multiProcessorCount;
        n = std::max(8, (ncu / 2) & ~7);
    }
    return n;
}

extern "C" int64_t papc_mlp_bwd_dw_max_ws_floats(int64_t M, int Cin, int Cout)
{
    (void)M;
    const int64_t n = (int64_t)(Cout + Cin) * Cin + Cin;
    return (int64_t)dw_max_chunks() * n + 2 * n + 2;
}

extern "C" int papc_mlp_bwd_dw_max_f32(const float *psel, const int32_t *argmax, int K, const float *x, const float *bn_scale, const float *bn_shift,
                                       const float *w, const float *e, const float *scale, const float *c1, int64_t M, int Cin, int Cout,
                                       float *workspace, float *dw, int accumulate, papc_stream_t stream)
{
    PAPC_REQUIRE(psel && argmax && x && bn_scale && bn_shift && w && e && scale && c1 && workspace && dw, PAPC_E_INVALID, "papc_mlp_bwd_dw_max_f32: null pointer");
    PAPC_REQUIRE(papc_mlp_max_nostore_ok(M, Cin, Cout, K), PAPC_E_UNSUPPORTED,
                 "papc_mlp_bwd_dw_max_f32: not built for M=%lld Cin=%d Cout=%d K=%d (see papc_mlp_max_nostore_ok)", (long long)M, Cin, Cout, K);
    PAPC_REQUIRE(aligned16(x) && aligned16(workspace), PAPC_E_INVALID, "papc_mlp_bwd_dw_max_f32: x / workspace must be 16-byte aligned");
    DwMaxArgs p;
    memset(&p, 0, sizeof(p));
    const int n = (Cout + Cin) * Cin + Cin;
    p.x = x; p.xsc = bn_scale; p.xsh = bn_shift; p.psel = psel; p.argmax = argmax; p.partial = workspace;
    p.M = M; p.part_ld = n; p.K = K; p.Cout = Cout; p.n_chunks = dw_max_chunks();
    p.rows_per_chunk = (int)(cdiv(cdiv(M, p.n_chunks), 64) * 64);
    double *fold = reinterpret_cast<double *>(workspace + (((int64_t)p.n_chunks * n + 1) & ~(int64_t)1));
    hipStream_t st = as_stream(stream);
    ProfScope prof(PAPC_K_BWD_DW, st);
    hipLaunchKernelGGL(dw_rows_max_kernel, dim3((unsigned)(2 * p.n_chunks)), dim3(512), 0, st, p);
    hipLaunchKernelGGL(dw_max_fold_kernel, dim3((unsigned)cdiv(n, 16)), dim3(64), 0, st, workspace, p.n_chunks, (int64_t)n, n, fold);
    hipLaunchKernelGGL(dw_max_finalize_kernel, dim3((unsigned)cdiv(Cout, 4)), dim3(256), 0, st, fold, w, e, scale, c1, 1.0 / (double)M, Cout, dw, accumulate);
    return check_launch("papc_mlp_bwd_dw_max_f32");
}
```

### papc_amd/csrc/sa_mlp.hip

```cpp
#include "common.h"

#define SA_CALL(expr)                 \
    do {                              \
        const int rc__ = (expr);      \
        if (rc__ != PAPC_OK) return rc__; \
    } while (0)

namespace papc {
int pfn_gram_stats(const float *features, const int32_t *num_voxels, const int32_t *coors, int P, int T, float vx, float vy, float x_offset, float y_offset, int zero_padded,
                   double *gram_partial, const float *w, int C, const float *gamma, const float *beta, float eps, float momentum, float *mean, float *invstd,
                   float *scale, float *shift, float *running_mean, float *running_var, double *gram, unsigned *ticket, hipStream_t st);
int pfn_gram_impl(const float *features, const int32_t *num_voxels, const int32_t *coors, int P, int T, float vx, float vy, float x_offset, float y_offset,
                  double *gram_partial, int zero_padded, papc_stream_t stream);
int pfn_apply_impl(const float *features, const int32_t *num_voxels, const int32_t *coors, int P, int T, float vx, float vy, float x_offset, float y_offset,
                   const float *w, int C, const float *scale, const float *shift, float *out, int32_t *argmax, int zero_padded, papc_stream_t stream);
int pfn_bwd_sparse_impl(const float *features, const int32_t *num_voxels, const int32_t *coors, int P, int T, float vx, float vy, float x_offset, float y_offset,
                        const float *w, int C, const float *gout, const int32_t *argmax, const float *mean, const float *invstd, const float *scale,
                        const float *shift, float *partial, int zero_padded, papc_stream_t stream);
int bn_finalize_clear(const float *stats_partial, int n_tiles, int64_t M, int C, const float *gamma, const float *beta, float eps, float momentum,
                      float *mean, float *invstd, float *scale, float *shift, float *running_mean, float *running_var, void *clr, int64_t bytes,
                      hipStream_t st);
int pfn_bwd_fold_finalize(const float *partial, int n_chunks, float *sums, int64_t M, const float *w, int C, const double *gram, const float *mean,
                          const float *invstd, const float *scale, float *dgamma, float *dbeta, float *dw, int flags, unsigned *ticket, hipStream_t st);

constexpr int A_PLAIN_ = PAPC_A_PLAIN, A_BNRELU_ = PAPC_A_BNRELU, A_GROUP_ = PAPC_A_GROUP, A_XYZ_ = PAPC_A_XYZ;

struct Carver {
    char *base;
    size_t off;
    template <class T>
    T *take(size_t n)
    {
        off = (off + 255) & ~(size_t)255;
        T *p = base ? reinterpret_cast<T *>(base + off) : nullptr;
        off += n * sizeof(T);
        return p;
    }
};

struct SavedPtrs {
    float *y[PAPC_SA_MAX_LAYERS];
    float *cst[PAPC_SA_MAX_LAYERS];
    int32_t *argmax;
    float *gbuf_f;
    float *xc; double *gram; float *wf;
    float *P;
};
struct FwdPtrs {
    float *stats;
    int32_t *gbuf_i;
    float *P, *wfeat;
    double *gpart;
    unsigned long long *keys;
};
struct BwdPtrs {
    float *c12[PAPC_SA_MAX_LAYERS];
    float *wt[PAPC_SA_MAX_LAYERS];
    float *part[PAPC_SA_MAX_LAYERS];
    float *red, *fused_red[2];
    float *dz[2];
    float *psel, *wcat, *hb, *eq, *dwmax_ws;
    float *bpart;
    float *dwx_part, *Gs, *part_g, *wft;
    float *tmp_gb;
};

static inline int64_t rows_of(const papc_sa_desc &d) { return (int64_t)d.B * d.S * d.K; }

static bool defer_fold(const papc_sa_grads &gr, const float *partial, int n_chunks, int64_t ld, int rows, int cols, float *out, int64_t out_ld, int accumulate)
{
    papc_fold_list *fl = gr.defer;
    if (!fl || !fl->jobs || fl->count >= fl->capacity) return false;
    papc_fold_job &j = fl->jobs[fl->count++];
    j.partial = partial; j.n_chunks = n_chunks; j.accumulate = accumulate; j.ld = ld; j.rows = rows; j.cols = cols; j.out = out; j.out_ld = out_ld;
    return true;
}
static bool defer_room(const papc_sa_grads &gr, int n) { return gr.defer && gr.defer->jobs && gr.defer->count + n <= gr.defer->capacity; }
static inline int cin_of(const papc_sa_plan &p, int l) { return l == 0 ? p.cin0 : p.d.cout[l - 1]; }
static inline bool seg_epi_widths(const papc_sa_plan &p)
{
    const int L = p.d.n_layers;
    return p.compact && p.d.pool && L >= 2 && cin_of(p, L - 1) == 128 && p.d.cout[L - 1] % 128 == 0;
}

static int dw_rows_per_chunk(int64_t M, int cout, int cin, int min_rows = 256)
{
    const bool wide = cin > 128 && cin <= 160;
    const int tiles = ((cout + 127) / 128) * (wide ? 1 : (cin + 127) / 128);
    const int want = std::max(1, 512 / tiles);
    int64_t rpc = (M + want - 1) / want;
    rpc = std::max<int64_t>(min_rows, ((rpc + 63) / 64) * 64);
    return (int)rpc;
}

static int dw_chunk(const papc_sa_plan &p, int l, int a_mode, int dz_mode)
{
    const int64_t M = rows_of(p.d);
    int rpc = 0;
    const bool plain = p.d.input == PAPC_SA_IN_ROWS;
    if (l > 0 || !plain) rpc = papc_mlp_bwd_dw_chunk_hint(M, cin_of(p, l), p.d.cout[l], a_mode, dz_mode, dz_mode == PAPC_DZ_MAX ? p.d.K : 0);
    if (rpc <= 0) rpc = dw_rows_per_chunk(M, p.d.cout[l], cin_of(p, l));
    return rpc;
}

static size_t layout_saved(const papc_sa_plan &p, void *base, SavedPtrs &s)
{
    Carver c{reinterpret_cast<char *>(base), 0};
    const int L = p.d.n_layers;
    const int64_t M = rows_of(p.d), G = (int64_t)p.d.B * p.d.S;
    memset(&s, 0, sizeof(s));
    for (int l = 0; l < L; ++l) {
        const bool stored = !(l == 0 && p.xyz1) && !(l == L - 1 && p.nostore);
        s.y[l] = stored ? c.take<float>((size_t)M * p.d.cout[l] + 64) : nullptr;
        s.cst[l] = c.take<float>(4 * (size_t)p.d.cout[l]);
    }
    if (p.d.pool) {
        s.argmax = c.take<int32_t>((size_t)G * p.d.cout[L - 1]);
        if (p.gmax || p.compact) s.gbuf_f = c.take<float>(2 * (size_t)G * p.d.cout[L - 1]);
    }
    if (p.xyz1) {
        s.xc = c.take<float>((size_t)M * 4);
        s.gram = c.take<double>(16);
        s.wf = c.take<float>(4 * (size_t)p.d.cout[0]);
    }
    if (p.lin0) s.P = c.take<float>((size_t)p.d.B * p.d.N * p.d.cout[0]);
    return c.off;
}

static size_t layout_fwd(const papc_sa_plan &p, void *base, FwdPtrs &f)
{
    Carver c{reinterpret_cast<char *>(base), 0};
    const int L = p.d.n_layers;
    const int64_t M = rows_of(p.d), G = (int64_t)p.d.B * p.d.S;
    memset(&f, 0, sizeof(f));
    int cmax = 0;
    for (int l = 0; l < L; ++l) cmax = std::max(cmax, p.d.cout[l]);
    const int rows = std::max(papc_mlp_gemm_parts(M), p.lin0 ? papc_lingather_parts(M) : 0) + (p.compact ? papc_compact_corr_parts() : 0);
    f.stats = c.take<float>((size_t)rows * 2 * cmax * L);
    if (p.gmax) f.gbuf_i = c.take<int32_t>(2 * (size_t)G * p.d.cout[L - 1]);
    if (p.lin0) f.wfeat = c.take<float>((size_t)p.d.cout[0] * p.d.D);
    if (p.xyz1) f.gpart = c.take<double>((size_t)papc_xyz_parts(M) * 16 + 16);
    if (seg_epi_widths(p)) f.keys = c.take<unsigned long long>((size_t)G * p.d.cout[L - 1]);
    return c.off;
}

static size_t layout_bwd(const papc_sa_plan &p, void *base, BwdPtrs &b)
{
    Carver c{reinterpret_cast<char *>(base), 0};
    const int L = p.d.n_layers;
    const int64_t M = rows_of(p.d), G = (int64_t)p.d.B * p.d.S;
    memset(&b, 0, sizeof(b));
    int cmax = p.cin0;
    for (int l = 0; l < L; ++l) cmax = std::max(cmax, p.d.cout[l]);
// ... 370 lines not shown
    SavedPtrs s; FwdPtrs f;
    layout_saved(p, io->saved, s);
    layout_fwd(p, io->scratch, f);
    const int parts = papc_mlp_gemm_parts(M);
    const bool wstats = p.compact && !(d.disable & PAPC_SA_NO_WSTATS);
    const int R_c = (p.compact && !wstats) ? papc_compact_corr_parts() : 0;
    papc_group_src grp;
    if (!plain) fill_grp(grp, d, *io, p.compact);
    if (!plain && wstats) grp.wstat = io->compact->wrow;
    int cmax = 0;
    for (int l = 0; l < L; ++l) cmax = std::max(cmax, d.cout[l]);
    const size_t stats_stride = (size_t)(std::max(parts, p.lin0 ? papc_lingather_parts(M) : 0) + R_c) * 2 * cmax;
    const bool seg_epi = seg_epi_widths(p) && !ev && knob(KNOB_SEG_EPI) && papc_mlp_seg_epi_ok(M, cin_of(p, L - 1), d.cout[L - 1]);

    const float *prev_y = nullptr, *prev_sc = nullptr, *prev_sh = nullptr;
    int cin = p.cin0;
    const float *xc = nullptr;
    papc_group_max gm;
    memset(&gm, 0, sizeof(gm));
    for (int l = 0; l < L; ++l) {
        const papc_sa_layer &ly = io->layer[l];
        PAPC_REQUIRE(ly.w && ly.gamma && ly.beta, PAPC_E_INVALID, "papc_sa_mlp_fwd: layer %d lacks w / gamma / beta", l);
        PAPC_REQUIRE(!ev || (ly.running_mean && ly.running_var), PAPC_E_INVALID, "papc_sa_mlp_fwd: eval_bn needs the running statistics");
        const int cout = d.cout[l];
        float *stats = ev ? nullptr : f.stats + (size_t)l * stats_stride;
        int parts_l = parts;
        const papc_group_max *gm_ref = nullptr;
        if (l == L - 1 && p.gmax) {
            gm.gmax = s.gbuf_f; gm.gmin = s.gbuf_f + G * cout; gm.amax = f.gbuf_i; gm.amin = f.gbuf_i + G * cout; gm.K = d.K;
            gm.sign_src = (d.disable & PAPC_SA_NO_GSIGN) ? nullptr : ly.gamma;
            gm_ref = &gm;
        }
        float *y = s.y[l];
        float *cst = s.cst[l];
        if (l == 0 && p.xyz1) {
            const double *gpart1;
            if (io->xc && io->xc_gram) { xc = io->xc; gpart1 = io->xc_gram; }
            else {
                SA_CALL(papc_xyz_group_f32(&grp, d.B, s.xc, f.gpart + 16, st));
                SA_CALL(papc_xyz_gram_fold_f32(f.gpart + 16, papc_xyz_parts(M), f.gpart, st));
                xc = s.xc; gpart1 = f.gpart;
            }
            SA_CALL(papc_xyz_l1_finalize_f32(gpart1, 1, M, ly.w, cin, 0, ly.b, ly.gamma, ly.beta, d.eps, d.momentum, cout, cst, cst + cout, cst + 2 * cout,
                                             cst + 3 * cout, ly.running_mean, ly.running_var, s.wf, s.gram, st));
            prev_y = nullptr; prev_sc = cst + 2 * cout; prev_sh = cst + 3 * cout;
            cin = cout;
            continue;
        }
        if (l == 1 && p.xyz1) {
            SA_CALL(papc_mlp_gemm_f32(A_XYZ_, xc, 4, nullptr, s.wf, nullptr, ly.w, ly.b, M, cin, cout, y, stats, gm_ref, st));
        } else if (l == 0 && plain) {
            SA_CALL(papc_mlp_gemm_f32(A_PLAIN_, io->x_rows, cin, nullptr, nullptr, nullptr, ly.w, ly.b, M, cin, cout, y, stats, gm_ref, st));
        } else if (l == 0 && p.lin0) {
            const int fcol0 = d.xyz_first ? 3 : 0;
            const float *wfeat = io->wfeat;
            if (!wfeat) {
                SA_CALL(papc_copy2d_f32(ly.w + fcol0, cin, f.wfeat, d.D, cout, d.D, 0, st));
                wfeat = f.wfeat;
            }
            const int64_t BN = (int64_t)d.B * d.N;
            SA_CALL(papc_mlp_gemm_f32(A_PLAIN_, io->feats, d.D, nullptr, nullptr, nullptr, wfeat, nullptr, BN, d.D, cout, s.P, nullptr, nullptr, st));
            parts_l = papc_lingather_parts(M);
            SA_CALL(papc_lingather_fwd_f32(s.P, &grp, d.B, ly.w, cin, d.xyz_first ? 0 : d.D, ly.b, cout, y, stats, st));
        } else if (l == 0) {
            SA_CALL(papc_mlp_gemm_f32(A_GROUP_, nullptr, 0, &grp, nullptr, nullptr, ly.w, ly.b, M, cin, cout, y, stats, gm_ref, st));
        } else if (p.compact && seg_epi && l == L - 1) {
            SA_CALL(papc_mlp_gemm_rows_keys_f32(prev_y, cin, prev_sc, prev_sh, ly.w, ly.b, M, cin, cout, y, stats, io->compact->rows,
                                                wstats ? io->compact->wrow : nullptr, io->compact->seg_grp, ly.gamma, f.keys, st));
        } else if (p.compact) {
            SA_CALL(papc_mlp_gemm_rows_w_f32(A_BNRELU_, prev_y, cin, nullptr, prev_sc, prev_sh, ly.w, ly.b, M, cin, cout, y, stats, nullptr, io->compact->rows,
                                             wstats ? io->compact->wrow : nullptr, st));
        } else {
            SA_CALL(papc_mlp_gemm_f32(A_BNRELU_, prev_y, cin, nullptr, prev_sc, prev_sh, ly.w, ly.b, M, cin, cout, y, stats, gm_ref, st));
        }
        if (p.compact && !wstats) {
            SA_CALL(papc_bn_stats_corr_f32(y, cout, io->compact->start, io->compact->coef, io->compact->G, stats + (size_t)parts_l * 2 * cout, st));
            parts_l += R_c;
        }
        if (ev) SA_CALL(papc_bn_eval_consts_f32(ly.running_mean, ly.running_var, ly.gamma, ly.beta, d.eps, cout, cst, cst + cout, cst + 2 * cout, cst + 3 * cout, st));
        else if (seg_epi && l == L - 2)
            SA_CALL(bn_finalize_clear(stats, parts_l, M, cout, ly.gamma, ly.beta, d.eps, d.momentum, cst, cst + cout, cst + 2 * cout, cst + 3 * cout,
                                      ly.running_mean, ly.running_var, f.keys, (int64_t)G * d.cout[L - 1] * 8, as_stream(st)));
        else SA_CALL(papc_bn_finalize_f32(stats, parts_l, M, cout, ly.gamma, ly.beta, d.eps, d.momentum, cst, cst + cout, cst + 2 * cout, cst + 3 * cout,
                                          ly.running_mean, ly.running_var, st));
        prev_y = y; prev_sc = cst + 2 * cout; prev_sh = cst + 3 * cout;
        cin = cout;
    }
    if (!d.pool) return papc_bn_relu_f32(prev_y, prev_sc, prev_sh, M, cin, io->out, st);
    if (p.compact && seg_epi)
        return papc_bn_relu_select_seg_f32(f.keys, prev_y, cin, io->compact->start, io->layer[L - 1].gamma, prev_sc, prev_sh, (int)G, io->out, s.argmax, s.gbuf_f, st);
    if (p.compact) return papc_bn_relu_max_seg_f32(prev_y, cin, io->compact->start, prev_sc, prev_sh, (int)G, io->out, s.argmax, s.gbuf_f, st);
    if (p.gmax) return papc_bn_select_max_f32(s.gbuf_f, s.gbuf_f + G * cin, f.gbuf_i, f.gbuf_i + G * cin, prev_sc, prev_sh, G, cin, io->out, s.argmax, st);
    return papc_bn_relu_max_f32(prev_y, prev_sc, prev_sh, G, d.K, cin, io->out, s.argmax, st);
}

int papc_sa_mlp_bwd(const papc_sa_plan *plan, const papc_sa_io *io, const papc_sa_grads *gr, papc_stream_t st)
{
    PAPC_REQUIRE(plan && io && gr && gr->gout && io->saved && io->scratch, PAPC_E_INVALID, "papc_sa_mlp_bwd: null pointer");
    const papc_sa_plan &p = *plan;
    const papc_sa_desc &d = p.d;
    const int L = d.n_layers;
    const int64_t M = rows_of(d), G = (int64_t)d.B * d.S;
    const bool plain = d.input == PAPC_SA_IN_ROWS, ev = d.eval_bn != 0;
    if (p.planes) return planes_bwd(p, *io, *gr, st);
    PAPC_REQUIRE(!ev || !(p.lin0 || p.xyz1 || p.nostore || p.sparse_max || p.compact || p.gmax), PAPC_E_INVALID,
                 "papc_sa_mlp_bwd: an eval_bn plan with a train-mode path set (lin0 %d xyz1 %d nostore %d sparse_max %d compact %d gmax %d)", p.lin0, p.xyz1,
                 p.nostore, p.sparse_max, p.compact, p.gmax);
    SavedPtrs s; BwdPtrs b;
    layout_saved(p, io->saved, s);
    layout_bwd(p, io->scratch, b);
    const float *xc = p.xyz1 ? ((io->xc && io->xc_gram) ? io->xc : s.xc) : nullptr;
    papc_group_src grp;
    if (!plain) fill_grp(grp, d, *io, p.compact);
    const int n_parts = (int)std::min<int64_t>(512, (M + 127) / 128);
    const int gemm_parts = papc_mlp_gemm_parts(M);
    const bool x_needs = plain && gr->grad_x, f_needs = !plain && d.D > 0 && gr->grad_feats && !d.cut_gather_grad;
    const float *ysel = (p.gmax || p.compact) ? s.gbuf_f : nullptr;
    const float *ones = io->consts3, *zeros = nullptr, *big = nullptr;
    int cmaxc = 0;
    for (int l = 0; l < L; ++l) cmaxc = std::max(cmaxc, d.cout[l]);
    if (p.lin0) {
        PAPC_REQUIRE(io->consts3 && io->consts3_ld >= d.cout[0], PAPC_E_INVALID, "papc_sa_mlp_bwd: the gather-add first layer needs consts3 (ones | zeros | 1e30 rows of >= %d floats)", d.cout[0]);
        zeros = io->consts3 + io->consts3_ld; big = io->consts3 + 2 * (int64_t)io->consts3_ld;
    }

    bool need_wt[PAPC_SA_MAX_LAYERS];
    const float *wts[PAPC_SA_MAX_LAYERS];
    for (int l = 0; l < L; ++l) {
        need_wt[l] = l > 0 || x_needs || f_needs;
        wts[l] = nullptr;
    }
    if (p.sparse_max) need_wt[L - 1] = false;
    if (p.lin0) need_wt[0] = false;
    {
        const float *srcs[8]; float *dsts[8]; int rws[8], cls[8];
        int n = 0;
        for (int l = 0; l < L; ++l) {
            if (!need_wt[l]) continue;
            if (gr->wt[l]) { wts[l] = gr->wt[l]; continue; }
            srcs[n] = io->layer[l].w; dsts[n] = b.wt[l]; rws[n] = d.cout[l]; cls[n] = cin_of(p, l);
            wts[l] = b.wt[l];
            if (++n == 8) { SA_CALL(papc_transpose_batch_f32(srcs, dsts, rws, cls, n, st)); n = 0; }
        }
        if (n) SA_CALL(papc_transpose_batch_f32(srcs, dsts, rws, cls, n, st));
    }

    papc_reduce_job jobs[PAPC_SA_MAX_LAYERS];
    int n_jobs = 0;
    bool xyz_fused = false;
    bool dz0_masked = false;
    const float *dz = nullptr;
    const float *fused_red = nullptr;
    int flip = 0;
    for (int l = L - 1; l >= 0; --l) {
        const papc_sa_layer &ly = io->layer[l];
        const int cout = d.cout[l], cin = cin_of(p, l);
        const float *cst = s.cst[l];
        float *c12 = b.c12[l];
        const bool acc_w = gr->acc_w[l] != 0, acc_gb = gr->acc_gb[l] != 0;
        float *dgamma = gr->dgamma[l] ? gr->dgamma[l] : b.tmp_gb, *dbeta = gr->dbeta[l] ? gr->dbeta[l] : b.tmp_gb + cmaxc;
        const bool gb_tmp = ev && acc_gb && gr->db[l];
        float *fgamma = gb_tmp ? b.tmp_gb : dgamma, *fbeta = gb_tmp ? b.tmp_gb + cmaxc : dbeta;
        PAPC_REQUIRE(gr->dw[l], PAPC_E_INVALID, "papc_sa_mlp_bwd: dw[%d] is NULL", l);
        papc_bwd_dy dy;
        memset(&dy, 0, sizeof(dy));
        if (p.compact) { dy.wrow = io->compact->wrow; dy.seg_grp = io->compact->seg_grp; dy.rows_dev = io->compact->rows; }
        if (l == L - 1 && !d.pool) { dy.dz_mode = PAPC_DZ_DENSE; dy.dz = gr->gout; dy.K = 1; }
        else if (l == L - 1) { dy.dz_mode = PAPC_DZ_MAX; dy.gout = gr->gout; dy.argmax = s.argmax; dy.K = d.K; }
        else { dy.dz_mode = PAPC_DZ_DENSE; dy.dz = dz; dy.K = 1; }
        if (l == 0 && p.xyz1) {
            PAPC_REQUIRE(!gr->dgamma[l] || (gr->acc_gb[l] != 0) == (gr->acc_w[l] != 0), PAPC_E_UNSUPPORTED,
                         "papc_sa_mlp_bwd: the coordinates-only first layer takes ONE accumulate flag for dw / dgamma / dbeta");
            int nbp = papc_xyz_bwd_parts(M);
            if (xyz_fused) nbp = papc_mlp_gemm_parts(M);
            else SA_CALL(papc_xyz_l1_bwd_f32(dz, xc, s.wf, M, cout, b.bpart, st));
            SA_CALL(papc_xyz_l1_bwd_finalize_f32(b.bpart, nbp, M, cout, s.gram, ly.w, cin, 0, ly.b, cst, cst + cout, cst + 2 * cout, dgamma, dbeta, gr->dw[l],
                                                 acc_w ? 1 : 0, st));
            if (gr->db[l] && !acc_w) SA_CALL(papc_fill_f32(gr->db[l], cout, 0.f, st));
            break;
        }
        dy.y = s.y[l];
        dy.mean = cst; dy.invstd = cst + cout; dy.scale = cst + 2 * cout; dy.shift = cst + 3 * cout;
        dy.c1 = c12; dy.c2 = c12 + cout;
        const float *red;
        int red_parts;
        if (!fused_red) {
            red = b.red; red_parts = n_parts;
            if (p.sparse_max && l == L - 1)
                SA_CALL(papc_bn_bwd_reduce_max_f32(ysel, dy.gout, dy.K, dy.mean, dy.invstd, dy.scale, dy.shift, M, cout, n_parts, b.red, b.psel, st));
            else if (p.compact && l == L - 1 && dy.dz_mode == PAPC_DZ_MAX && ysel && b.psel && !(d.disable & PAPC_SA_NO_PSEL)) {
                SA_CALL(papc_bn_bwd_reduce_max_f32(ysel, dy.gout, dy.K, dy.mean, dy.invstd, dy.scale, dy.shift, M, cout, n_parts, b.red, b.psel, st));
                dy.psel = b.psel;
            } else
                SA_CALL(papc_bn_bwd_reduce_f32(dy.dz_mode, dy.dz_mode == PAPC_DZ_MAX ? ysel : dy.dz, dy.gout, dy.argmax, dy.K, dy.y, dy.mean, dy.invstd, dy.scale,
                                               dy.shift, M, cout, n_parts, b.red, st));
        } else { red = fused_red; red_parts = gemm_parts; }
        SA_CALL(papc_bn_bwd_finalize_f32(red, red_parts, M, cout, fgamma, fbeta, c12, c12 + cout, ((acc_gb && !gb_tmp) ? 1 : 0) | (ev ? 2 : 0), st));
        if (l == 0 && p.lin0) {
            const int64_t BN = (int64_t)d.B * d.N;
            const int parts_l = papc_lingather_bwd_parts(&grp, d.B, cout);
            if (!papc_lingather_bwd_lists_ok(&grp, cout)) SA_CALL(papc_fill_f32(b.Gs, BN * cout, 0.f, st));
            if (dz0_masked && papc_lingather_bwd_pp_ok(&grp, d.B, cout))
                SA_CALL(papc_lingather_bwd_pp_f32(&dy, &grp, d.B, cout, s.P, ly.w, cin, d.xyz_first ? 0 : d.D, ly.b, b.Gs, b.dwx_part, st));
            else
                SA_CALL(papc_lingather_bwd_f32(&dy, &grp, d.B, cout, b.Gs, b.dwx_part, st));
            const int fcol0 = d.xyz_first ? 3 : 0, xcol0 = d.xyz_first ? 0 : d.D;
            float *dw = gr->dw[l];
            const int acc = acc_w ? 1 : 0;
            if (!defer_fold(*gr, b.dwx_part, parts_l, (int64_t)cout * 3, cout, 3, dw + xcol0, cin, acc))
                SA_CALL(papc_reduce_partials_strided_f32(b.dwx_part, parts_l, (int64_t)cout * 3, cout, 3, dw + xcol0, cin, acc, st));
            papc_bwd_dy dyg;
            memset(&dyg, 0, sizeof(dyg));
            dyg.dz_mode = PAPC_DZ_DENSE; dyg.dz = b.Gs; dyg.K = 1; dyg.y = b.Gs;
            dyg.mean = zeros; dyg.invstd = ones; dyg.scale = ones; dyg.shift = big; dyg.c1 = zeros; dyg.c2 = zeros;
            const int rpc_g = dw_rows_per_chunk(BN, cout, d.D, 64);
            const int n_chunks_g = (int)((BN + rpc_g - 1) / rpc_g);
            const int64_t pld_g = (int64_t)cout * d.D + cout;
            SA_CALL(papc_mlp_bwd_dw_f32(&dyg, A_PLAIN_, io->feats, d.D, nullptr, nullptr, nullptr, BN, d.D, cout, rpc_g, b.part_g, b.part_g + (int64_t)cout * d.D, pld_g, st));
            if (!defer_fold(*gr, b.part_g, n_chunks_g, pld_g, cout, d.D, dw + fcol0, cin, acc))
                SA_CALL(papc_reduce_partials_strided_f32(b.part_g, n_chunks_g, pld_g, cout, d.D, dw + fcol0, cin, acc, st));
            if (gr->db[l] && !acc_w) SA_CALL(papc_fill_f32(gr->db[l], cout, 0.f, st));
            if (f_needs) {
                const float *wft;
                if (gr->wt[l]) wft = gr->wt[l] + (int64_t)fcol0 * cout;
                else {
                    SA_CALL(papc_copy2d_f32(ly.w + fcol0, cin, b.wft, cout, cout, d.D, 1, st));
                    wft = b.wft;
                }
                SA_CALL(papc_mlp_gemm_f32(A_PLAIN_, b.Gs, cout, nullptr, nullptr, nullptr, wft, nullptr, BN, cout, d.D, gr->grad_feats, nullptr, nullptr, st));
            }
            break;
        }
        if (p.sparse_max && l == L - 1) {
            SA_CALL(papc_bn_max_prep_f32(nullptr, nullptr, cst + 2 * cout, cst + 3 * cout, cst, cst + cout, c12, c12 + cout, ly.w, ly.b, G, cout, cin, nullptr,
                                         b.wcat, b.hb, b.eq, b.eq + cout, st));
        }
        const bool x1 = p.xyz1 && l == 1;
        if (p.nostore && l == L - 1) {
            const float *pc = s.cst[l - 1];
            SA_CALL(papc_mlp_bwd_dw_max_f32(b.psel, s.argmax, d.K, s.y[l - 1], pc + 2 * cin, pc + 3 * cin, ly.w, b.eq, cst + 2 * cout, c12, M, cin, cout, b.dwmax_ws,
                                            gr->dw[l], acc_w ? 1 : 0, st));
            if (gr->db[l] && !acc_w) SA_CALL(papc_fill_f32(gr->db[l], cout, 0.f, st));
        } else {
            const int am = l == 0 ? (plain ? A_PLAIN_ : A_GROUP_) : (x1 ? A_XYZ_ : A_BNRELU_);
            const int rpc = dw_chunk(p, l, am, dy.dz_mode);
            const int n_chunks = (int)((M + rpc - 1) / rpc);
            const int64_t pld = (int64_t)cout * cin + cout;
            float *dwp = b.part[l], *dbp = b.part[l] + (int64_t)cout * cin;
            if (l == 0 && plain) SA_CALL(papc_mlp_bwd_dw_f32(&dy, A_PLAIN_, io->x_rows, cin, nullptr, nullptr, nullptr, M, cin, cout, rpc, dwp, dbp, pld, st));
            else if (l == 0) SA_CALL(papc_mlp_bwd_dw_f32(&dy, A_GROUP_, nullptr, 0, &grp, nullptr, nullptr, M, cin, cout, rpc, dwp, dbp, pld, st));
            else if (x1) SA_CALL(papc_mlp_bwd_dw_f32(&dy, A_XYZ_, xc, 4, nullptr, s.wf, nullptr, M, cin, cout, rpc, dwp, dbp, pld, st));
            else {
                const float *pc = s.cst[l - 1];
                SA_CALL(papc_mlp_bwd_dw_f32(&dy, A_BNRELU_, s.y[l - 1], cin, nullptr, pc + 2 * cin, pc + 3 * cin, M, cin, cout, rpc, dwp, dbp, pld, st));
            }
            const bool want_db = gr->db[l] && !ev;
            if (defer_room(*gr, 2)) {
                defer_fold(*gr, b.part[l], n_chunks, pld, 1, cout * cin, gr->dw[l], (int64_t)cout * cin, acc_w ? 1 : 0);
                if (want_db) defer_fold(*gr, b.part[l] + (int64_t)cout * cin, n_chunks, pld, 1, cout, gr->db[l], cout, acc_w ? 1 : 0);
            } else {
                papc_reduce_job &j = jobs[n_jobs++];
                j.partial = b.part[l]; j.n_chunks = n_chunks; j.accumulate = acc_w ? 1 : 0; j.ld = pld; j.n1 = (int64_t)cout * cin; j.out1 = gr->dw[l];
                j.n2 = want_db ? cout : 0; j.out2 = want_db ? gr->db[l] : nullptr;
            }
            if (ev && gr->db[l]) {
                hipLaunchKernelGGL(mul_vec_kernel, dim3((unsigned)cdiv(cout, 256)), dim3(256), 0, as_stream(st), cst + 2 * cout, fbeta, cout, gr->db[l], acc_w ? 1 : 0);
                SA_CALL(check_launch("papc_sa_mlp_bwd (eval-mode bias gradient)"));
                if (gb_tmp) {
                    hipLaunchKernelGGL(add_vec2_kernel, dim3((unsigned)cdiv(cout, 256)), dim3(256), 0, as_stream(st), fgamma, fbeta, cout, gr->dgamma[l], gr->dbeta[l]);
                    SA_CALL(check_launch("papc_sa_mlp_bwd (eval-mode dgamma / dbeta accumulate)"));
                }
            }
        }
        fused_red = nullptr;
        if (l > 0) {
            float *dz_prev = b.dz[flip];
            flip ^= (b.dz[1] ? 1 : 0);
            papc_bwd_red nr;
            const papc_bwd_red *nr_ref = nullptr;
            if (!(d.disable & PAPC_SA_NO_FUSED_RED) && !x1) {
                const float *pc = s.cst[l - 1];
                nr.y = s.y[l - 1]; nr.mean = pc; nr.invstd = pc + cin; nr.scale = pc + 2 * cin; nr.shift = pc + 3 * cin;
                float *fr = b.fused_red[l & 1];
                nr.red_partial = fr;
                nr.store_masked = 0;
                if (l == 1 && p.lin0 && papc_lingather_bwd_pp_ok(&grp, d.B, p.d.cout[0])) {
                    nr.store_masked = 1;
                    dz0_masked = true;
                }
                nr_ref = &nr;
                fused_red = fr;
            }
            if (p.sparse_max && l == L - 1) {
                const float *pc = s.cst[l - 1];
                SA_CALL(papc_mlp_bwd_dx_max_f32(b.psel, s.argmax, d.K, s.y[l - 1], cin, pc + 2 * cin, pc + 3 * cin, b.wcat, b.hb, M, cin, cout, dz_prev, nr_ref, st));
            } else {
                if (x1 && !(d.disable & PAPC_SA_NO_XYZ_FUSE) && dy.dz_mode == PAPC_DZ_DENSE && !dy.wrow && papc_mlp_bwd_dx_xyz_ok(M, cin, cout)) {
                    const int rc = papc_mlp_bwd_dx_xyz_f32(&dy, wts[l], M, cin, cout, xc, s.wf, b.bpart, st);
                    if (rc == PAPC_OK) xyz_fused = true;
                    else if (rc != PAPC_E_UNSUPPORTED) return rc;
                }
                if (!xyz_fused) SA_CALL(papc_mlp_bwd_dx_f32(&dy, wts[l], M, cin, cout, dz_prev, nullptr, nr_ref, st));
            }
            dz = dz_prev;
        } else if (x_needs) {
            SA_CALL(papc_mlp_bwd_dx_f32(&dy, wts[l], M, cin, cout, gr->grad_x, nullptr, nullptr, st));
        } else if (f_needs) {
            SA_CALL(papc_fill_f32(gr->grad_feats, (int64_t)d.B * d.N * d.D, 0.f, st));
            papc_scatter_dst sc;
            memset(&sc, 0, sizeof(sc));
            sc.grad_feats = gr->grad_feats; sc.idx = io->idx; sc.N = d.N; sc.S = d.S; sc.K = d.K; sc.D = d.D; sc.col0 = d.xyz_first ? 3 : 0;
            SA_CALL(papc_mlp_bwd_dx_f32(&dy, wts[l], M, cin, cout, nullptr, &sc, nullptr, st));
        }
    }
    if (n_jobs) SA_CALL(papc_reduce_partials_batch_f32(jobs, n_jobs, st));
    return PAPC_OK;
}

static void pfn_layout(const papc_pfn_desc &d, void *saved, void *scratch, float *&cst, int32_t *&argmax, double *&gram, double *&gpart, float *&part, float *&sums)
{
    Carver cs{reinterpret_cast<char *>(saved), 0};
    cst = cs.take<float>(4 * (size_t)d.C);
    argmax = cs.take<int32_t>((size_t)d.P * d.C);
    gram = cs.take<double>(256);
    Carver cw{reinterpret_cast<char *>(scratch), 0};
    gpart = cw.take<double>((size_t)papc_pfn_gram_blocks(d.P) * 256);
    part = cw.take<float>((size_t)papc_pfn_num_blocks(d.P) * 11 * d.C);
    sums = cw.take<float>(11 * (size_t)d.C);
}

int papc_pfn_workspace(const papc_pfn_desc *desc, int64_t *saved_bytes, int64_t *scratch_bytes)
{
    PAPC_REQUIRE(desc && saved_bytes && scratch_bytes, PAPC_E_INVALID, "papc_pfn_workspace: null pointer");
    PAPC_REQUIRE(desc->P >= 1 && desc->T >= 1 && desc->C >= 1 && desc->C <= 64, PAPC_E_UNSUPPORTED, "papc_pfn_workspace: P=%d T=%d C=%d (C in 1..64)", desc->P, desc->T, desc->C);
    const papc_pfn_desc &d = *desc;
    *saved_bytes = 256 + ((4 * (int64_t)d.C * 4 + 255) & ~255ll) + (((int64_t)d.P * d.C * 4 + 255) & ~255ll) + 2048;
    *scratch_bytes = 256 + (((int64_t)papc_pfn_gram_blocks(d.P) * 2048 + 255) & ~255ll) + (((int64_t)papc_pfn_num_blocks(d.P) * 11 * d.C * 4 + 255) & ~255ll) + 11 * d.C * 4 + 256;
    return PAPC_OK;
}

int papc_pfn_fwd(const papc_pfn_desc *desc, const papc_pfn_io *io, papc_stream_t st)
{
    PAPC_REQUIRE(desc && io && io->features && io->num_voxels && io->coors && io->w && io->out && io->saved && io->scratch, PAPC_E_INVALID, "papc_pfn_fwd: null pointer");
    const papc_pfn_desc &d = *desc;
    float *cst, *part, *sums; int32_t *argmax; double *gram, *gpart;
    pfn_layout(d, io->saved, io->scratch, cst, argmax, gram, gpart, part, sums);
    const int C = d.C;
    if (d.training) {
        const int ng = papc_pfn_gram_blocks(d.P);
        unsigned *tk = knob(KNOB_PFN_FUSED_TAILS) ? io->tickets : nullptr;
        if (tk) {
            SA_CALL(papc::pfn_gram_stats(io->features, io->num_voxels, io->coors, d.P, d.T, d.vx, d.vy, d.x_offset, d.y_offset, d.zero_padded, gpart, io->w, C, io->gamma, io->beta,
                                         d.eps, d.momentum, cst, cst + C, cst + 2 * C, cst + 3 * C, io->running_mean, io->running_var, gram, tk, as_stream(st)));
        } else {
            SA_CALL(papc::pfn_gram_impl(io->features, io->num_voxels, io->coors, d.P, d.T, d.vx, d.vy, d.x_offset, d.y_offset, gpart, d.zero_padded, st));
            SA_CALL(papc_pfn_gram_finalize_f32(gpart, ng, (int64_t)d.P * d.T, io->w, C, io->gamma, io->beta, d.eps, d.momentum, cst, cst + C, cst + 2 * C, cst + 3 * C,
                                               io->running_mean, io->running_var, gram, st));
        }
    } else {
        PAPC_REQUIRE(io->running_mean && io->running_var, PAPC_E_INVALID, "papc_pfn_fwd: eval mode needs the running statistics");
        SA_CALL(papc_bn_eval_consts_f32(io->running_mean, io->running_var, io->gamma, io->beta, d.eps, C, cst, cst + C, cst + 2 * C, cst + 3 * C, st));
    }
    return papc::pfn_apply_impl(io->features, io->num_voxels, io->coors, d.P, d.T, d.vx, d.vy, d.x_offset, d.y_offset, io->w, C, cst + 2 * C, cst + 3 * C, io->out, argmax, d.zero_padded, st);
}

int papc_pfn_bwd(const papc_pfn_desc *desc, const papc_pfn_io *io, const float *gout, float *dw, float *dgamma, float *dbeta, int accumulate, papc_stream_t st)
{
    PAPC_REQUIRE(desc && io && io->features && io->num_voxels && io->coors && io->w && io->saved && io->scratch && gout && dw && dgamma && dbeta, PAPC_E_INVALID,
                 "papc_pfn_bwd: null pointer");
    const papc_pfn_desc &d = *desc;
    float *cst, *part, *sums; int32_t *argmax; double *gram, *gpart;
    pfn_layout(d, io->saved, io->scratch, cst, argmax, gram, gpart, part, sums);
    const int C = d.C, nb = papc_pfn_num_blocks(d.P);
    if (!d.training) SA_CALL(papc_fill_f32(reinterpret_cast<float *>(gram), 512, 0.f, st));
    SA_CALL(papc::pfn_bwd_sparse_impl(io->features, io->num_voxels, io->coors, d.P, d.T, d.vx, d.vy, d.x_offset, d.y_offset, io->w, C, gout, argmax, cst, cst + C,
                                      cst + 2 * C, cst + 3 * C, part, d.zero_padded, st));
    unsigned *tk = knob(KNOB_PFN_FUSED_TAILS) ? io->tickets : nullptr;
    if (tk)
        return papc::pfn_bwd_fold_finalize(part, nb, sums, (int64_t)d.P * d.T, io->w, C, gram, cst, cst + C, cst + 2 * C, dgamma, dbeta, dw,
                                           (d.training ? 0 : 1) | (accumulate ? 2 : 0), tk + 1, as_stream(st));
    SA_CALL(papc_reduce_partials_f32(part, nb, 11 * (int64_t)C, sums, 0, st));
    return papc_pfn_bwd_finalize_f32(sums, (int64_t)d.P * d.T, io->w, C, gram, cst, cst + C, cst + 2 * C, dgamma, dbeta, dw, (d.training ? 0 : 1) | (accumulate ? 2 : 0), st);
}

}
```

Before: 22310.

## Carry BN backward finalize and max-fold work as tail jobs in dW kernels

```diff
diff --git a/papc_amd/csrc/bn_fold.h b/papc_amd/csrc/bn_fold.h
--- /dev/null
+++ b/papc_amd/csrc/bn_fold.h
@@ -0,0 +1,60 @@
+#pragma once
+#include "common.h"
+
+namespace papc {
+
+template <int D>
+__device__ __forceinline__ void sum_partial_rows_d(const float *__restrict__ part, int n_tiles, int C, int c, int tl, double &s1, double &s2)
+{
+    for (int t0 = tl; t0 < n_tiles; t0 += 64 * D) {
+        float a[D], b[D];
+#pragma unroll
+        for (int j = 0; j < D; ++j) {
+            const int t = t0 + 64 * j;
+            const int64_t o = (int64_t)(t < n_tiles ? t : t0) * 2 * C + c;
+            a[j] = part[o];
+            b[j] = part[o + C];
+        }
+#pragma unroll
+        for (int j = 0; j < D; ++j) {
+            if (t0 + 64 * j < n_tiles) { s1 += (double)a[j]; s2 += (double)b[j]; }
+        }
+    }
+}
+__device__ __forceinline__ void sum_partial_rows(const float *__restrict__ part, int n_tiles, int C, int c, int tl, double &s1, double &s2)
+{
+    if (n_tiles > 512) sum_partial_rows_d<16>(part, n_tiles, C, c, tl, s1, s2);
+    else sum_partial_rows_d<8>(part, n_tiles, C, c, tl, s1, s2);
+}
+
+__device__ __forceinline__ double lane_get(double v, int l)
+{
+    const int lo = __builtin_amdgcn_readlane(__double2loint(v), l), hi = __builtin_amdgcn_readlane(__double2hiint(v), l);
+    return __hiloint2double(hi, lo);
+}
+__device__ __forceinline__ void fold_part_lanes(double &s1, double &s2)
+{
+    s1 += __shfl_xor(s1, 1); s2 += __shfl_xor(s2, 1);
+    s1 += __shfl_xor(s1, 2); s2 += __shfl_xor(s2, 2);
+    double t1 = 0.0, t2 = 0.0;
+#pragma unroll
+    for (int w = 0; w < 16; ++w) { t1 += lane_get(s1, 4 * w); t2 += lane_get(s2, 4 * w); }
+    s1 = t1; s2 = t2;
+}
+
+__device__ __forceinline__ void bn_bwd_finalize_channel(const float *__restrict__ part, int n_tiles, int64_t M, int C, float *dgamma, float *dbeta,
+                                                        float *c1, float *c2, int accumulate, int c, int tl)
+{
+    double s1 = 0.0, s2 = 0.0;
+    sum_partial_rows(part, n_tiles, C, c, tl, s1, s2);
+    fold_part_lanes(s1, s2);
+    if (tl == 0) {
+        if (dbeta) dbeta[c] = (accumulate & 1) ? dbeta[c] + (float)s1 : (float)s1;
+        if (dgamma) dgamma[c] = (accumulate & 1) ? dgamma[c] + (float)s2 : (float)s2;
+        const bool eval_bn = (accumulate & 2) != 0;
+        c1[c] = eval_bn ? 0.f : (float)(s1 / (double)M);
+        c2[c] = eval_bn ? 0.f : (float)(s2 / (double)M);
+    }
+}
+
+}
diff --git a/papc_amd/csrc/bn_ops.hip b/papc_amd/csrc/bn_ops.hip
--- a/papc_amd/csrc/bn_ops.hip
+++ b/papc_amd/csrc/bn_ops.hip
@@ -1,4 +1,4 @@
-#include "common.h"
+#include "bn_fold.h"
 
 namespace papc {
 
@@ -17,45 +17,6 @@
     __device__ float &operator[](int) { return v; }
     __device__ float operator[](int) const { return v; }
 };
-
-template <int D>
-__device__ __forceinline__ void sum_partial_rows_d(const float *__restrict__ part, int n_tiles, int C, int c, int tl, double &s1, double &s2)
-{
-    for (int t0 = tl; t0 < n_tiles; t0 += 64 * D) {
-        float a[D], b[D];
-#pragma unroll
-        for (int j = 0; j < D; ++j) {
-            const int t = t0 + 64 * j;
-            const int64_t o = (int64_t)(t < n_tiles ? t : t0) * 2 * C + c;
-            a[j] = part[o];
-            b[j] = part[o + C];
-        }
-#pragma unroll
-        for (int j = 0; j < D; ++j) {
-            if (t0 + 64 * j < n_tiles) { s1 += (double)a[j]; s2 += (double)b[j]; }
-        }
-    }
-}
-__device__ __forceinline__ void sum_partial_rows(const float *__restrict__ part, int n_tiles, int C, int c, int tl, double &s1, double &s2)
-{
-    if (n_tiles > 512) sum_partial_rows_d<16>(part, n_tiles, C, c, tl, s1, s2);
-    else sum_partial_rows_d<8>(part, n_tiles, C, c, tl, s1, s2);
-}
-
-__device__ __forceinline__ double lane_get(double v, int l)
-{
-    const int lo = __builtin_amdgcn_readlane(__double2loint(v), l), hi = __builtin_amdgcn_readlane(__double2hiint(v), l);
-    return __hiloint2double(hi, lo);
-}
-__device__ __forceinline__ void fold_part_lanes(double &s1, double &s2)
-{
-    s1 += __shfl_xor(s1, 1); s2 += __shfl_xor(s2, 1);
-    s1 += __shfl_xor(s1, 2); s2 += __shfl_xor(s2, 2);
-    double t1 = 0.0, t2 = 0.0;
-#pragma unroll
-    for (int w = 0; w < 16; ++w) { t1 += lane_get(s1, 4 * w); t2 += lane_get(s2, 4 * w); }
-    s1 = t1; s2 = t2;
-}
 
 __device__ __forceinline__ void bn_finalize_channel(const int c, const float *__restrict__ part, int n_tiles, int64_t M, int C,
                                                     const float *__restrict__ gamma, const float *__restrict__ beta,
@@ -250,17 +211,7 @@
 __global__ __launch_bounds__(64) void bn_bwd_finalize_kernel(const float *__restrict__ part, int n_tiles, int64_t M, int C,
                                                             float *dgamma, float *dbeta, float *c1, float *c2, int accumulate)
 {
-    const int c = blockIdx.x, tl = threadIdx.x;
-    double s1 = 0.0, s2 = 0.0;
-    sum_partial_rows(part, n_tiles, C, c, tl, s1, s2);
-    fold_part_lanes(s1, s2);
-    if (tl == 0) {
-        if (dbeta) dbeta[c] = (accumulate & 1) ? dbeta[c] + (float)s1 : (float)s1;
-        if (dgamma) dgamma[c] = (accumulate & 1) ? dgamma[c] + (float)s2 : (float)s2;
-        const bool eval_bn = (accumulate & 2) != 0;
-        c1[c] = eval_bn ? 0.f : (float)(s1 / (double)M);
-        c2[c] = eval_bn ? 0.f : (float)(s2 / (double)M);
-    }
+    bn_bwd_finalize_channel(part, n_tiles, M, C, dgamma, dbeta, c1, c2, accumulate, blockIdx.x, threadIdx.x);
 }
 
 __global__ void bn_eval_consts_kernel(const float *__restrict__ rmean, const float *__restrict__ rvar, const float *__restrict__ gamma,
diff --git a/papc_amd/csrc/capi.hip b/papc_amd/csrc/capi.hip
--- a/papc_amd/csrc/capi.hip
+++ b/papc_amd/csrc/capi.hip
@@ -71,6 +71,7 @@
     {"PAPC_PG_GROUP", 1, 0, 1},
     {"PAPC_PG_PIPE", 1, 0, 1},
     {"PAPC_SEG_EPI", 1, 0, 1},
+    {"PAPC_BWD_TAILJOBS", 1, 0, 2},
 };
 static int g_knobs[KNOB_COUNT];
 static int knob_parse(int id, const char *e)
diff --git a/papc_amd/csrc/common.h b/papc_amd/csrc/common.h
--- a/papc_amd/csrc/common.h
+++ b/papc_amd/csrc/common.h
@@ -24,7 +24,7 @@
 enum Knob {
     KNOB_LG_PARTS, KNOB_DW_F32, KNOB_DW_DBG, KNOB_DW_XYZ, KNOB_PARTS, KNOB_GEMM_F32, KNOB_GEMM_WAVES, KNOB_MAXCAT_WAVES,
     KNOB_GEMM_WS, KNOB_GEMM_OCC, KNOB_GEMM_DBG, KNOB_GEMM_KB, KNOB_GEMM_MINWG, KNOB_GEMM_TL, KNOB_FPS_THREADS,
-    KNOB_FPS_THREADS_SMALL, KNOB_STREAM, KNOB_STREAM_MINTILES, KNOB_STREAM_CK, KNOB_STREAM_ASM, KNOB_PFN_MFMA, KNOB_DW_RS64, KNOB_DW_ROWS, KNOB_DW_ROWS_BLOCKS, KNOB_DW_ROWSX, KNOB_PG_DBG, KNOB_PG_NB, KNOB_PG_NS, KNOB_STREAM_MAXCAT, KNOB_MAX_NOSTORE, KNOB_PFN_FUSED_TAILS, KNOB_STREAM_NW12, KNOB_LG_LISTS, KNOB_FOLD_WAVES, KNOB_LGL_VARIANT, KNOB_LG_PP, KNOB_PG_GROUP, KNOB_PG_PIPE, KNOB_SEG_EPI, KNOB_COUNT
+    KNOB_FPS_THREADS_SMALL, KNOB_STREAM, KNOB_STREAM_MINTILES, KNOB_STREAM_CK, KNOB_STREAM_ASM, KNOB_PFN_MFMA, KNOB_DW_RS64, KNOB_DW_ROWS, KNOB_DW_ROWS_BLOCKS, KNOB_DW_ROWSX, KNOB_PG_DBG, KNOB_PG_NB, KNOB_PG_NS, KNOB_STREAM_MAXCAT, KNOB_MAX_NOSTORE, KNOB_PFN_FUSED_TAILS, KNOB_STREAM_NW12, KNOB_LG_LISTS, KNOB_FOLD_WAVES, KNOB_LGL_VARIANT, KNOB_LG_PP, KNOB_PG_GROUP, KNOB_PG_PIPE, KNOB_SEG_EPI, KNOB_BWD_TAILJOBS, KNOB_COUNT
 };
 int knob(int id);
 
diff --git a/papc_amd/csrc/dw_tail.h b/papc_amd/csrc/dw_tail.h
--- /dev/null
+++ b/papc_amd/csrc/dw_tail.h
@@ -0,0 +1,59 @@
+#pragma once
+#include "bn_fold.h"
+
+namespace papc {
+
+enum { DW_TAIL_BN_FINALIZE = 1, DW_TAIL_MAX_FOLD = 2 };
+
+struct DwTail {
+    int kind;
+    int n_units;
+    const float *red; int red_parts, C, accumulate; int64_t M;
+    float *dgamma, *dbeta, *c1, *c2;
+    const float *fpart; int f_chunks, f_n; int64_t f_ld; double *f_out;
+};
+
+inline int dw_tail_bn_units(const DwTail &t) { return (t.kind & DW_TAIL_BN_FINALIZE) ? t.C : 0; }
+inline int dw_tail_fold_units(const DwTail &t) { return (t.kind & DW_TAIL_MAX_FOLD) ? (t.f_n + 15) / 16 : 0; }
+
+__device__ __forceinline__ void dw_max_fold_unit(const float *__restrict__ partial, int n_chunks, int64_t part_ld, int n, double *__restrict__ out, int u, int tl)
+{
+    const int l = tl & 15, q = tl >> 4;
+    const int e = u * 16 + l;
+    const int per = (n_chunks + 3) / 4, c0 = q * per, c1 = min(n_chunks, c0 + per);
+    double s = 0.0;
+    if (e < n) {
+        int c = c0;
+        for (; c + 8 <= c1; c += 8) {
+            float v[8];
+#pragma unroll
+            for (int j = 0; j < 8; ++j) v[j] = partial[(int64_t)(c + j) * part_ld + e];
+#pragma unroll
+            for (int j = 0; j < 8; ++j) s += (double)v[j];
+        }
+        for (; c < c1; ++c) s += (double)partial[(int64_t)c * part_ld + e];
+    }
+    const double s1 = __shfl(s, l + 16), s2 = __shfl(s, l + 32), s3 = __shfl(s, l + 48);
+    if (q == 0 && e < n) out[e] = ((s + s1) + s2) + s3;
+}
+
+__device__ __forceinline__ void dw_tail_run(const DwTail &t, int wg_flat, int n_wg, int waves, int wave, int lane)
+{
+    const int nbn = (t.kind & DW_TAIL_BN_FINALIZE) ? t.C : 0;
+    for (int u = __builtin_amdgcn_readfirstlane(wave) * n_wg + wg_flat; u < t.n_units; u += n_wg * waves) {
+        if (u < nbn) bn_bwd_finalize_channel(t.red, t.red_parts, t.M, t.C, t.dgamma, t.dbeta, t.c1, t.c2, t.accumulate, u, lane);
+        else dw_max_fold_unit(t.fpart, t.f_chunks, t.f_ld, t.f_n, t.f_out, u - nbn, lane);
+    }
+}
+
+int mlp_bwd_dw_tail(const papc_bwd_dy *dy, int a_mode, const float *x, int64_t ldx, const papc_group_src *grp, const float *bn_scale, const float *bn_shift,
+                    int64_t M, int Cin, int Cout, int rows_per_chunk, float *dw_partial, float *db_partial, int64_t part_ld, const DwTail *tail,
+                    papc_stream_t stream);
+int mlp_bwd_dw_max_rows(const float *psel, const int32_t *argmax, int K, const float *x, const float *bn_scale, const float *bn_shift, const float *w,
+                        const float *e, const float *scale, const float *c1, int64_t M, int Cin, int Cout, float *workspace, float *dw, int accumulate,
+                        const DwTail *tail, int fold_now, DwTail *fold_job, papc_stream_t stream);
+int mlp_bwd_dw_max_fold(const DwTail *fold_job, papc_stream_t stream);
+int mlp_bwd_dw_max_finish(const float *w, const float *e, const float *scale, const float *c1, int64_t M, int Cin, int Cout, float *workspace, float *dw,
+                          int accumulate, papc_stream_t stream);
+
+}
diff --git a/papc_amd/csrc/mlp_dw.hip b/papc_amd/csrc/mlp_dw.hip
--- a/papc_amd/csrc/mlp_dw.hip
+++ b/papc_amd/csrc/mlp_dw.hip
@@ -1,5 +1,6 @@
 #include <type_traits>
 #include "mlp_loaders.h"
+#include "dw_tail.h"
 
 namespace papc {
 
@@ -28,6 +29,7 @@
     int TOp, TIp;
     int RS;
     unsigned long long *dbg;
+    DwTail tail;
 };
 
 constexpr int DW_T = 128;
@@ -694,6 +696,7 @@
                 }
     }
     if (p.db_partial && blockIdx.z == 0 && tid < 64) p.db_partial[(int64_t)blockIdx.x * p.part_ld + o0 + tid] = 0.f;
+    if (p.tail.kind) dw_tail_run(p.tail, (int)(blockIdx.x + gridDim.x * (blockIdx.y + gridDim.y * blockIdx.z)), (int)(gridDim.x * gridDim.y * gridDim.z), 8, wave, lane);
 }
 
 template <int DYMODE, int NW, bool CP = false, bool RG = false>
@@ -947,6 +950,7 @@
             out[(int64_t)c * CI + 32 * b + l31] = acc[b][r];
         }
     if (p.db_partial && tid < CB && (!RG || (blockIdx.z == 0 && (int)blockIdx.y * CB + tid < p.Cout))) p.db_partial[(int64_t)blockIdx.x * p.part_ld + blockIdx.y * CB + tid] = 0.f;
+    if (p.tail.kind) dw_tail_run(p.tail, (int)(blockIdx.x + gridDim.x * (blockIdx.y + gridDim.y * blockIdx.z)), (int)(gridDim.x * gridDim.y * gridDim.z), NW, wave, lane);
 }
 
 static unsigned long long *g_dw_dbg = nullptr;
@@ -956,6 +960,7 @@
     float *partial;
     int64_t M, part_ld;
     int K, Cout, rows_per_chunk, n_chunks;
+    DwTail tail;
 };
 
 __global__ __launch_bounds__(512, 2) void dw_rows_max_kernel(DwMaxArgs p)
@@ -1109,27 +1114,12 @@
                     out[(int64_t)row * CI + 32 * b + l31] = acc[a][b][r];
                 }
     }
+    if (p.tail.kind) dw_tail_run(p.tail, (int)blockIdx.x, (int)gridDim.x, 8, wave, lane);
 }
 
 __global__ __launch_bounds__(64) void dw_max_fold_kernel(const float *__restrict__ partial, int n_chunks, int64_t part_ld, int n, double *__restrict__ out)
 {
-    const int l = threadIdx.x & 15, q = threadIdx.x >> 4;
-    const int e = blockIdx.x * 16 + l;
-    const int per = (n_chunks + 3) / 4, c0 = q * per, c1 = min(n_chunks, c0 + per);
-    double s = 0.0;
-    if (e < n) {
-        int c = c0;
-        for (; c + 8 <= c1; c += 8) {
-            float v[8];
-#pragma unroll
-            for (int j = 0; j < 8; ++j) v[j] = partial[(int64_t)(c + j) * part_ld + e];
-#pragma unroll
-            for (int j = 0; j < 8; ++j) s += (double)v[j];
-        }
-        for (; c < c1; ++c) s += (double)partial[(int64_t)c * part_ld + e];
-    }
-    const double s1 = __shfl(s, l + 16), s2 = __shfl(s, l + 32), s3 = __shfl(s, l + 48);
-    if (q == 0 && e < n) out[e] = ((s + s1) + s2) + s3;
+    dw_max_fold_unit(partial, n_chunks, part_ld, n, out, (int)blockIdx.x, (int)threadIdx.x);
 }
 
 __global__ __launch_bounds__(256) void dw_max_finalize_kernel(const double *__restrict__ fold, const float *__restrict__ w, const float *__restrict__ e,
@@ -1178,7 +1168,7 @@
 }
 
 template <int XMODE, int DYMODE, bool VEC>
-static int launch_dw_v(const DwArgs &p_in, hipStream_t st)
+static int launch_dw_v(const DwArgs &p_in, hipStream_t st, bool *carried)
 {
     DwArgs p = p_in;
     const int dbg_on = knob(KNOB_DW_DBG);
@@ -1207,6 +1197,7 @@
             dim3 g2((unsigned)cdiv(p.M, p.rows_per_chunk), (unsigned)(p.Cout / 128));
             hipLaunchKernelGGL((dw_rowsx_kernel<DYMODE, 4, true>), g2, dim3(256), 0, st, p);
         }
+        *carried = true;
         return check_launch("papc_mlp_bwd_dw_f32 (compacted)");
     }
     if (VEC && XMODE == A_BNRELU && rowsx_rows_ok && dw_rowsx_eligible(p.Cin, p.Cout, DYMODE == A_DY_DENSE, p.dy.d.K) && p.x.ldx == p.Cin && p.rows_per_chunk % 16 == 0 &&
@@ -1224,12 +1215,14 @@
             dim3 g2((unsigned)cdiv(p.M, p.rows_per_chunk), (unsigned)(p.Cout / 128));
             hipLaunchKernelGGL((dw_rowsx_kernel<DYMODE, 4>), g2, dim3(256), 0, st, p);
         }
+        *carried = true;
         return check_launch("papc_mlp_bwd_dw_f32");
     }
     const bool rows_rows_ok = p.M % 16 == 0 && p.M * (int64_t)std::max(p.Cout, p.Cin) * 4 < (1ll << 32);
     if (VEC && XMODE == A_BNRELU && rows_rows_ok && dw_rows_eligible(p.Cin, p.Cout, DYMODE == A_DY_DENSE, p.dy.d.K) && p.x.ldx == p.Cin && p.rows_per_chunk % 16 == 0) {
         dim3 g2((unsigned)cdiv(p.M, p.rows_per_chunk), (unsigned)(p.Cout / 64), (unsigned)(p.Cin / 64));
         hipLaunchKernelGGL((dw_rows_kernel<DYMODE>), g2, dim3(512), 0, st, p);
+        *carried = true;
         return check_launch("papc_mlp_bwd_dw_f32");
     }
     if (VEC && XMODE != A_GROUP && !wide && to >= 2 && ti >= 2 && off32 && k4 && !dw_f32_exact()) {
@@ -1253,9 +1246,9 @@
 }
 
 template <int XMODE, int DYMODE>
-static int launch_dw(const DwArgs &p, bool vec, hipStream_t st)
-{
-    return vec ? launch_dw_v<XMODE, DYMODE, true>(p, st) : launch_dw_v<XMODE, DYMODE, false>(p, st);
+static int launch_dw(const DwArgs &p, bool vec, hipStream_t st, bool *carried)
+{
+    return vec ? launch_dw_v<XMODE, DYMODE, true>(p, st, carried) : launch_dw_v<XMODE, DYMODE, false>(p, st, carried);
 }
 
 static int pad_tile(int c) { return c <= 32 ? 32 : (c <= 64 ? 64 : 128); }
@@ -1285,10 +1278,19 @@
     return (int)std::min<int64_t>(rpc, 1 << 24);
 }
 
-extern "C" int papc_mlp_bwd_dw_f32(const papc_bwd_dy *dy, int a_mode, const float *x, int64_t ldx,
-                                   const papc_group_src *grp, const float *bn_scale, const float *bn_shift, int64_t M,
-                                   int Cin, int Cout, int rows_per_chunk, float *dw_partial, float *db_partial,
-                                   int64_t part_ld, papc_stream_t stream)
+static int dw_tail_launches(const DwTail &t, papc_stream_t stream)
+{
+    if (t.kind & DW_TAIL_BN_FINALIZE) {
+        const int rc = papc_bn_bwd_finalize_f32(t.red, t.red_parts, t.M, t.C, t.dgamma, t.dbeta, t.c1, t.c2, t.accumulate, stream);
+        if (rc) return rc;
+    }
+    if (t.kind & DW_TAIL_MAX_FOLD) return mlp_bwd_dw_max_fold(&t, stream);
+    return PAPC_OK;
+}
+
+static int dw_entry(const papc_bwd_dy *dy, int a_mode, const float *x, int64_t ldx, const papc_group_src *grp, const float *bn_scale, const float *bn_shift,
+                    int64_t M, int Cin, int Cout, int rows_per_chunk, float *dw_partial, float *db_partial, int64_t part_ld, const DwTail *tail,
+                    bool *carried, papc_stream_t stream)
 {
     PAPC_REQUIRE(dw_partial, PAPC_E_INVALID, "papc_mlp_bwd_dw_f32: null dw_partial");
     PAPC_REQUIRE(M >= 1 && Cin >= 1 && Cout >= 1, PAPC_E_INVALID, "papc_mlp_bwd_dw_f32: bad sizes");
@@ -1301,6 +1303,7 @@
     if (rc) return rc;
     DwArgs p;
     memset(&p, 0, sizeof(p));
+    if (tail) p.tail = *tail;
     rc = fill_asrc(p.x, a_mode, x, ldx, grp, bn_scale, bn_shift, Cin, "papc_mlp_bwd_dw_f32");
     if (rc) return rc;
     if (a_mode == A_XYZ) {
@@ -1316,6 +1319,7 @@
         dim3 g2((unsigned)cdiv(M, rows_per_chunk), (unsigned)(Cout / 64), (unsigned)(Cin / 64));
         if (dense_) hipLaunchKernelGGL((dw_rows_kernel<A_DY_DENSE, true>), g2, dim3(512), 0, st2, p);
         else hipLaunchKernelGGL((dw_rows_kernel<A_DY_MAX, true>), g2, dim3(512), 0, st2, p);
+        *carried = true;
         return check_launch("papc_mlp_bwd_dw_f32");
     }
     fill_dy(p.dy.d, dy);
@@ -1336,10 +1340,30 @@
         return check_launch("papc_mlp_bwd_dw_f32");
     }
     switch (a_mode) {
-    case A_PLAIN: return dense ? launch_dw<A_PLAIN, A_DY_DENSE>(p, vec, st) : launch_dw<A_PLAIN, A_DY_MAX>(p, vec, st);
-    case A_BNRELU: return dense ? launch_dw<A_BNRELU, A_DY_DENSE>(p, vec, st) : launch_dw<A_BNRELU, A_DY_MAX>(p, vec, st);
-    default: return dense ? launch_dw<A_GROUP, A_DY_DENSE>(p, vec, st) : launch_dw<A_GROUP, A_DY_MAX>(p, vec, st);
-    }
+    case A_PLAIN: return dense ? launch_dw<A_PLAIN, A_DY_DENSE>(p, vec, st, carried) : launch_dw<A_PLAIN, A_DY_MAX>(p, vec, st, carried);
+    case A_BNRELU: return dense ? launch_dw<A_BNRELU, A_DY_DENSE>(p, vec, st, carried) : launch_dw<A_BNRELU, A_DY_MAX>(p, vec, st, carried);
+    default: return dense ? launch_dw<A_GROUP, A_DY_DENSE>(p, vec, st, carried) : launch_dw<A_GROUP, A_DY_MAX>(p, vec, st, carried);
+    }
+}
+
+extern "C" int papc_mlp_bwd_dw_f32(const papc_bwd_dy *dy, int a_mode, const float *x, int64_t ldx,
+                                   const papc_group_src *grp, const float *bn_scale, const float *bn_shift, int64_t M,
+                                   int Cin, int Cout, int rows_per_chunk, float *dw_partial, float *db_partial,
+                                   int64_t part_ld, papc_stream_t stream)
+{
+    bool carried = false;
+    return dw_entry(dy, a_mode, x, ldx, grp, bn_scale, bn_shift, M, Cin, Cout, rows_per_chunk, dw_partial, db_partial, part_ld, nullptr, &carried, stream);
+}
+
+int papc::mlp_bwd_dw_tail(const papc_bwd_dy *dy, int a_mode, const float *x, int64_t ldx, const papc_group_src *grp, const float *bn_scale, const float *bn_shift,
+                          int64_t M, int Cin, int Cout, int rows_per_chunk, float *dw_partial, float *db_partial, int64_t part_ld, const DwTail *tail,
+                          papc_stream_t stream)
+{
+    if (tail && !tail->kind) tail = nullptr;
+    bool carried = false;
+    const int rc = dw_entry(dy, a_mode, x, ldx, grp, bn_scale, bn_shift, M, Cin, Cout, rows_per_chunk, dw_partial, db_partial, part_ld, tail, &carried, stream);
+    if (rc || !tail || carried) return rc;
+    return dw_tail_launches(*tail, stream);
 }
 
 static int dw_max_chunks()
@@ -1361,25 +1385,61 @@
     return (int64_t)dw_max_chunks() * n + 2 * n + 2;
 }
 
-extern "C" int papc_mlp_bwd_dw_max_f32(const float *psel, const int32_t *argmax, int K, const float *x, const float *bn_scale, const float *bn_shift,
-                                       const float *w, const float *e, const float *scale, const float *c1, int64_t M, int Cin, int Cout,
-                                       float *workspace, float *dw, int accumulate, papc_stream_t stream)
+int papc::mlp_bwd_dw_max_rows(const float *psel, const int32_t *argmax, int K, const float *x, const float *bn_scale, const float *bn_shift, const float *w,
+                              const float *e, const float *scale, const float *c1, int64_t M, int Cin, int Cout, float *workspace, float *dw, int accumulate,
+                              const DwTail *tail, int fold_now, DwTail *fold_job, papc_stream_t stream)
 {
     PAPC_REQUIRE(psel && argmax && x && bn_scale && bn_shift && w && e && scale && c1 && workspace && dw, PAPC_E_INVALID, "papc_mlp_bwd_dw_max_f32: null pointer");
     PAPC_REQUIRE(papc_mlp_max_nostore_ok(M, Cin, Cout, K), PAPC_E_UNSUPPORTED,
                  "papc_mlp_bwd_dw_max_f32: not built for M=%lld Cin=%d Cout=%d K=%d (see papc_mlp_max_nostore_ok)", (long long)M, Cin, Cout, K);
     PAPC_REQUIRE(aligned16(x) && aligned16(workspace), PAPC_E_INVALID, "papc_mlp_bwd_dw_max_f32: x / workspace must be 16-byte aligned");
+    PAPC_REQUIRE(fold_now || fold_job, PAPC_E_INVALID, "papc_mlp_bwd_dw_max_f32: a deferred fold needs its descriptor");
     DwMaxArgs p;
     memset(&p, 0, sizeof(p));
     const int n = (Cout + Cin) * Cin + Cin;
     p.x = x; p.xsc = bn_scale; p.xsh = bn_shift; p.psel = psel; p.argmax = argmax; p.partial = workspace;
     p.M = M; p.part_ld = n; p.K = K; p.Cout = Cout; p.n_chunks = dw_max_chunks();
     p.rows_per_chunk = (int)(cdiv(cdiv(M, p.n_chunks), 64) * 64);
-    double *fold = reinterpret_cast<double *>(workspace + (((int64_t)p.n_chunks * n + 1) & ~(int64_t)1));
+    if (tail && tail->kind) p.tail = *tail;
+    DwTail fj;
+    memset(&fj, 0, sizeof(fj));
+    fj.kind = DW_TAIL_MAX_FOLD;
+    fj.fpart = workspace; fj.f_chunks = p.n_chunks; fj.f_n = n; fj.f_ld = n;
+    fj.f_out = reinterpret_cast<double *>(workspace + (((int64_t)p.n_chunks * n + 1) & ~(int64_t)1));
+    fj.n_units = dw_tail_fold_units(fj);
+    if (fold_job) *fold_job = fj;
     hipStream_t st = as_stream(stream);
     ProfScope prof(PAPC_K_BWD_DW, st);
     hipLaunchKernelGGL(dw_rows_max_kernel, dim3((unsigned)(2 * p.n_chunks)), dim3(512), 0, st, p);
-    hipLaunchKernelGGL(dw_max_fold_kernel, dim3((unsigned)cdiv(n, 16)), dim3(64), 0, st, workspace, p.n_chunks, (int64_t)n, n, fold);
+    if (fold_now) {
+        hipLaunchKernelGGL(dw_max_fold_kernel, dim3((unsigned)cdiv(n, 16)), dim3(64), 0, st, workspace, p.n_chunks, (int64_t)n, n, fj.f_out);
+        hipLaunchKernelGGL(dw_max_finalize_kernel, dim3((unsigned)cdiv(Cout, 4)), dim3(256), 0, st, fj.f_out, w, e, scale, c1, 1.0 / (double)M, Cout, dw, accumulate);
+    }
+    return check_launch("papc_mlp_bwd_dw_max_f32");
+}
+
+int papc::mlp_bwd_dw_max_fold(const DwTail *fj, papc_stream_t stream)
+{
+    hipStream_t st = as_stream(stream);
+    ProfScope prof(PAPC_K_BWD_DW, st);
+    hipLaunchKernelGGL(dw_max_fold_kernel, dim3((unsigned)cdiv(fj->f_n, 16)), dim3(64), 0, st, fj->fpart, fj->f_chunks, fj->f_ld, fj->f_n, fj->f_out);
+    return check_launch("papc_mlp_bwd_dw_max_f32 (fold)");
+}
+
+int papc::mlp_bwd_dw_max_finish(const float *w, const float *e, const float *scale, const float *c1, int64_t M, int Cin, int Cout, float *workspace, float *dw,
+                                int accumulate, papc_stream_t stream)
+{
+    const int n = (Cout + Cin) * Cin + Cin;
+    const double *fold = reinterpret_cast<const double *>(workspace + (((int64_t)dw_max_chunks() * n + 1) & ~(int64_t)1));
+    hipStream_t st = as_stream(stream);
+    ProfScope prof(PAPC_K_BWD_DW, st);
     hipLaunchKernelGGL(dw_max_finalize_kernel, dim3((unsigned)cdiv(Cout, 4)), dim3(256), 0, st, fold, w, e, scale, c1, 1.0 / (double)M, Cout, dw, accumulate);
-    return check_launch("papc_mlp_bwd_dw_max_f32");
-}
+    return check_launch("papc_mlp_bwd_dw_max_f32 (finalize)");
+}
+
+extern "C" int papc_mlp_bwd_dw_max_f32(const float *psel, const int32_t *argmax, int K, const float *x, const float *bn_scale, const float *bn_shift,
+                                       const float *w, const float *e, const float *scale, const float *c1, int64_t M, int Cin, int Cout,
+                                       float *workspace, float *dw, int accumulate, papc_stream_t stream)
+{
+    return mlp_bwd_dw_max_rows(psel, argmax, K, x, bn_scale, bn_shift, w, e, scale, c1, M, Cin, Cout, workspace, dw, accumulate, nullptr, 1, nullptr, stream);
+}
diff --git a/papc_amd/csrc/sa_mlp.hip b/papc_amd/csrc/sa_mlp.hip
--- a/papc_amd/csrc/sa_mlp.hip
+++ b/papc_amd/csrc/sa_mlp.hip
@@ -1,4 +1,5 @@
 #include "common.h"
+#include "dw_tail.h"
 
 #define SA_CALL(expr)                 \
     do {                              \
@@ -675,6 +676,11 @@
     const float *dz = nullptr;
     const float *fused_red = nullptr;
     int flip = 0;
+    const bool tj = knob(KNOB_BWD_TAILJOBS) != 0 && !ev, carry = knob(KNOB_BWD_TAILJOBS) == 1;
+    bool fin_carried = false;
+    bool fold_pending = false;
+    DwTail fold_job;
+    memset(&fold_job, 0, sizeof(fold_job));
     for (int l = L - 1; l >= 0; --l) {
         const papc_sa_layer &ly = io->layer[l];
         const int cout = d.cout[l], cin = cin_of(p, l);
@@ -718,7 +724,9 @@
                 SA_CALL(papc_bn_bwd_reduce_f32(dy.dz_mode, dy.dz_mode == PAPC_DZ_MAX ? ysel : dy.dz, dy.gout, dy.argmax, dy.K, dy.y, dy.mean, dy.invstd, dy.scale,
                                                dy.shift, M, cout, n_parts, b.red, st));
         } else { red = fused_red; red_parts = gemm_parts; }
-        SA_CALL(papc_bn_bwd_finalize_f32(red, red_parts, M, cout, fgamma, fbeta, c12, c12 + cout, ((acc_gb && !gb_tmp) ? 1 : 0) | (ev ? 2 : 0), st));
+        if (!fin_carried)
+            SA_CALL(papc_bn_bwd_finalize_f32(red, red_parts, M, cout, fgamma, fbeta, c12, c12 + cout, ((acc_gb && !gb_tmp) ? 1 : 0) | (ev ? 2 : 0), st));
+        fin_carried = false;
         if (l == 0 && p.lin0) {
             const int64_t BN = (int64_t)d.B * d.N;
             const int parts_l = papc_lingather_bwd_parts(&grp, d.B, cout);
@@ -759,82 +767,127 @@
                                          b.wcat, b.hb, b.eq, b.eq + cout, st));
         }
         const bool x1 = p.xyz1 && l == 1;
-        if (p.nostore && l == L - 1) {
-            const float *pc = s.cst[l - 1];
-            SA_CALL(papc_mlp_bwd_dw_max_f32(b.psel, s.argmax, d.K, s.y[l - 1], pc + 2 * cin, pc + 3 * cin, ly.w, b.eq, cst + 2 * cout, c12, M, cin, cout, b.dwmax_ws,
-                                            gr->dw[l], acc_w ? 1 : 0, st));
-            if (gr->db[l] && !acc_w) SA_CALL(papc_fill_f32(gr->db[l], cout, 0.f, st));
-        } else {
-            const int am = l == 0 ? (plain ? A_PLAIN_ : A_GROUP_) : (x1 ? A_XYZ_ : A_BNRELU_);
-            const int rpc = dw_chunk(p, l, am, dy.dz_mode);
-            const int n_chunks = (int)((M + rpc - 1) / rpc);
-            const int64_t pld = (int64_t)cout * cin + cout;
-            float *dwp = b.part[l], *dbp = b.part[l] + (int64_t)cout * cin;
-            if (l == 0 && plain) SA_CALL(papc_mlp_bwd_dw_f32(&dy, A_PLAIN_, io->x_rows, cin, nullptr, nullptr, nullptr, M, cin, cout, rpc, dwp, dbp, pld, st));
-            else if (l == 0) SA_CALL(papc_mlp_bwd_dw_f32(&dy, A_GROUP_, nullptr, 0, &grp, nullptr, nullptr, M, cin, cout, rpc, dwp, dbp, pld, st));
-            else if (x1) SA_CALL(papc_mlp_bwd_dw_f32(&dy, A_XYZ_, xc, 4, nullptr, s.wf, nullptr, M, cin, cout, rpc, dwp, dbp, pld, st));
-            else {
+        auto run_dw = [&](const DwTail *tail) -> int {
+            if (p.nostore && l == L - 1) {
                 const float *pc = s.cst[l - 1];
-                SA_CALL(papc_mlp_bwd_dw_f32(&dy, A_BNRELU_, s.y[l - 1], cin, nullptr, pc + 2 * cin, pc + 3 * cin, M, cin, cout, rpc, dwp, dbp, pld, st));
-            }
-            const bool want_db = gr->db[l] && !ev;
-            if (defer_room(*gr, 2)) {
-                defer_fold(*gr, b.part[l], n_chunks, pld, 1, cout * cin, gr->dw[l], (int64_t)cout * cin, acc_w ? 1 : 0);
-                if (want_db) defer_fold(*gr, b.part[l] + (int64_t)cout * cin, n_chunks, pld, 1, cout, gr->db[l], cout, acc_w ? 1 : 0);
+                if (!tj)
+                    SA_CALL(papc_mlp_bwd_dw_max_f32(b.psel, s.argmax, d.K, s.y[l - 1], pc + 2 * cin, pc + 3 * cin, ly.w, b.eq, cst + 2 * cout, c12, M, cin, cout, b.dwmax_ws,
+                                                    gr->dw[l], acc_w ? 1 : 0, st));
+                else {
+                    const bool below = l - 1 > 0 || (l - 1 == 0 && !p.xyz1 && !p.lin0);
+                    SA_CALL(mlp_bwd_dw_max_rows(b.psel, s.argmax, d.K, s.y[l - 1], pc + 2 * cin, pc + 3 * cin, ly.w, b.eq, cst + 2 * cout, c12, M, cin, cout, b.dwmax_ws,
+                                                gr->dw[l], acc_w ? 1 : 0, tail, below ? 0 : 1, &fold_job, st));
+                    fold_pending = below;
+                }
+                if (gr->db[l] && !acc_w) SA_CALL(papc_fill_f32(gr->db[l], cout, 0.f, st));
             } else {
-                papc_reduce_job &j = jobs[n_jobs++];
-                j.partial = b.part[l]; j.n_chunks = n_chunks; j.accumulate = acc_w ? 1 : 0; j.ld = pld; j.n1 = (int64_t)cout * cin; j.out1 = gr->dw[l];
-                j.n2 = want_db ? cout : 0; j.out2 = want_db ? gr->db[l] : nullptr;
-            }
-            if (ev && gr->db[l]) {
-                hipLaunchKernelGGL(mul_vec_kernel, dim3((unsigned)cdiv(cout, 256)), dim3(256), 0, as_stream(st), cst + 2 * cout, fbeta, cout, gr->db[l], acc_w ? 1 : 0);
-                SA_CALL(check_launch("papc_sa_mlp_bwd (eval-mode bias gradient)"));
-                if (gb_tmp) {
-                    hipLaunchKernelGGL(add_vec2_kernel, dim3((unsigned)cdiv(cout, 256)), dim3(256), 0, as_stream(st), fgamma, fbeta, cout, gr->dgamma[l], gr->dbeta[l]);
-                    SA_CALL(check_launch("papc_sa_mlp_bwd (eval-mode dgamma / dbeta accumulate)"));
+                const int am = l == 0 ? (plain ? A_PLAIN_ : A_GROUP_) : (x1 ? A_XYZ_ : A_BNRELU_);
+                const int rpc = dw_chunk(p, l, am, dy.dz_mode);
+                const int n_chunks = (int)((M + rpc - 1) / rpc);
+                const int64_t pld = (int64_t)cout * cin + cout;
+                float *dwp = b.part[l], *dbp = b.part[l] + (int64_t)cout * cin;
+                if (l == 0 && plain) SA_CALL(mlp_bwd_dw_tail(&dy, A_PLAIN_, io->x_rows, cin, nullptr, nullptr, nullptr, M, cin, cout, rpc, dwp, dbp, pld, tail, st));
+                else if (l == 0) SA_CALL(mlp_bwd_dw_tail(&dy, A_GROUP_, nullptr, 0, &grp, nullptr, nullptr, M, cin, cout, rpc, dwp, dbp, pld, tail, st));
+                else if (x1) SA_CALL(mlp_bwd_dw_tail(&dy, A_XYZ_, xc, 4, nullptr, s.wf, nullptr, M, cin, cout, rpc, dwp, dbp, pld, tail, st));
+                else {
+                    const float *pc = s.cst[l - 1];
+                    SA_CALL(mlp_bwd_dw_tail(&dy, A_BNRELU_, s.y[l - 1], cin, nullptr, pc + 2 * cin, pc + 3 * cin, M, cin, cout, rpc, dwp, dbp, pld, tail, st));
+                }
+                const bool want_db = gr->db[l] && !ev;
+                if (defer_room(*gr, 2)) {
+                    defer_fold(*gr, b.part[l], n_chunks, pld, 1, cout * cin, gr->dw[l], (int64_t)cout * cin, acc_w ? 1 : 0);
+                    if (want_db) defer_fold(*gr, b.part[l] + (int64_t)cout * cin, n_chunks, pld, 1, cout, gr->db[l], cout, acc_w ? 1 : 0);
+                } else {
+                    papc_reduce_job &j = jobs[n_jobs++];
+                    j.partial = b.part[l]; j.n_chunks = n_chunks; j.accumulate = acc_w ? 1 : 0; j.ld = pld; j.n1 = (int64_t)cout * cin; j.out1 = gr->dw[l];
+                    j.n2 = want_db ? cout : 0; j.out2 = want_db ? gr->db[l] : nullptr;
+                }
+                if (ev && gr->db[l]) {
+                    hipLaunchKernelGGL(mul_vec_kernel, dim3((unsigned)cdiv(cout, 256)), dim3(256), 0, as_stream(st), cst + 2 * cout, fbeta, cout, gr->db[l], acc_w ? 1 : 0);
+                    SA_CALL(check_launch("papc_sa_mlp_bwd (eval-mode bias gradient)"));
+                    if (gb_tmp) {
+                        hipLaunchKernelGGL(add_vec2_kernel, dim3((unsigned)cdiv(cout, 256)), dim3(256), 0, as_stream(st), fgamma, fbeta, cout, gr->dgamma[l], gr->dbeta[l]);
+                        SA_CALL(check_launch("papc_sa_mlp_bwd (eval-mode dgamma / dbeta accumulate)"));
+                    }
                 }
             }
-        }
-        fused_red = nullptr;
-        if (l > 0) {
-            float *dz_prev = b.dz[flip];
-            flip ^= (b.dz[1] ? 1 : 0);
-            papc_bwd_red nr;
-            const papc_bwd_red *nr_ref = nullptr;
-            if (!(d.disable & PAPC_SA_NO_FUSED_RED) && !x1) {
-                const float *pc = s.cst[l - 1];
-                nr.y = s.y[l - 1]; nr.mean = pc; nr.invstd = pc + cin; nr.scale = pc + 2 * cin; nr.shift = pc + 3 * cin;
-                float *fr = b.fused_red[l & 1];
-                nr.red_partial = fr;
-                nr.store_masked = 0;
-                if (l == 1 && p.lin0 && papc_lingather_bwd_pp_ok(&grp, d.B, p.d.cout[0])) {
-                    nr.store_masked = 1;
-                    dz0_masked = true;
+            return PAPC_OK;
+        };
+        auto run_dx = [&]() -> int {
+            fused_red = nullptr;
+            if (l > 0) {
+                float *dz_prev = b.dz[flip];
+                flip ^= (b.dz[1] ? 1 : 0);
+                papc_bwd_red nr;
+                const papc_bwd_red *nr_ref = nullptr;
+                if (!(d.disable & PAPC_SA_NO_FUSED_RED) && !x1) {
+                    const float *pc = s.cst[l - 1];
+                    nr.y = s.y[l - 1]; nr.mean = pc; nr.invstd = pc + cin; nr.scale = pc + 2 * cin; nr.shift = pc + 3 * cin;
+                    float *fr = b.fused_red[l & 1];
+                    nr.red_partial = fr;
+                    nr.store_masked = 0;
+                    if (l == 1 && p.lin0 && papc_lingather_bwd_pp_ok(&grp, d.B, p.d.cout[0])) {
+                        nr.store_masked = 1;
+                        dz0_masked = true;
+                    }
+                    nr_ref = &nr;
+                    fused_red = fr;
                 }
-                nr_ref = &nr;
-                fused_red = fr;
+                if (p.sparse_max && l == L - 1) {
+                    const float *pc = s.cst[l - 1];
+                    SA_CALL(papc_mlp_bwd_dx_max_f32(b.psel, s.argmax, d.K, s.y[l - 1], cin, pc + 2 * cin, pc + 3 * cin, b.wcat, b.hb, M, cin, cout, dz_prev, nr_ref, st));
+                } else {
+                    if (x1 && !(d.disable & PAPC_SA_NO_XYZ_FUSE) && dy.dz_mode == PAPC_DZ_DENSE && !dy.wrow && papc_mlp_bwd_dx_xyz_ok(M, cin, cout)) {
+                        const int rc = papc_mlp_bwd_dx_xyz_f32(&dy, wts[l], M, cin, cout, xc, s.wf, b.bpart, st);
+                        if (rc == PAPC_OK) xyz_fused = true;
+                        else if (rc != PAPC_E_UNSUPPORTED) return rc;
+                    }
+                    if (!xyz_fused) SA_CALL(papc_mlp_bwd_dx_f32(&dy, wts[l], M, cin, cout, dz_prev, nullptr, nr_ref, st));
+                }
+                dz = dz_prev;
+            } else if (x_needs) {
+                SA_CALL(papc_mlp_bwd_dx_f32(&dy, wts[l], M, cin, cout, gr->grad_x, nullptr, nullptr, st));
+            } else if (f_needs) {
+                SA_CALL(papc_fill_f32(gr->grad_feats, (int64_t)d.B * d.N * d.D, 0.f, st));
+                papc_scatter_dst sc;
+                memset(&sc, 0, sizeof(sc));
+                sc.grad_feats = gr->grad_feats; sc.idx = io->idx; sc.N = d.N; sc.S = d.S; sc.K = d.K; sc.D = d.D; sc.col0 = d.xyz_first ? 3 : 0;
+                SA_CALL(papc_mlp_bwd_dx_f32(&dy, wts[l], M, cin, cout, nullptr, &sc, nullptr, st));
             }
-            if (p.sparse_max && l == L - 1) {
-                const float *pc = s.cst[l - 1];
-                SA_CALL(papc_mlp_bwd_dx_max_f32(b.psel, s.argmax, d.K, s.y[l - 1], cin, pc + 2 * cin, pc + 3 * cin, b.wcat, b.hb, M, cin, cout, dz_prev, nr_ref, st));
-            } else {
-                if (x1 && !(d.disable & PAPC_SA_NO_XYZ_FUSE) && dy.dz_mode == PAPC_DZ_DENSE && !dy.wrow && papc_mlp_bwd_dx_xyz_ok(M, cin, cout)) {
-                    const int rc = papc_mlp_bwd_dx_xyz_f32(&dy, wts[l], M, cin, cout, xc, s.wf, b.bpart, st);
-                    if (rc == PAPC_OK) xyz_fused = true;
-                    else if (rc != PAPC_E_UNSUPPORTED) return rc;
-                }
-                if (!xyz_fused) SA_CALL(papc_mlp_bwd_dx_f32(&dy, wts[l], M, cin, cout, dz_prev, nullptr, nr_ref, st));
+            return PAPC_OK;
+        };
+        DwTail tail;
+        memset(&tail, 0, sizeof(tail));
+        const bool dx_first = tj && l > 0;
+        if (dx_first) {
+            SA_CALL(run_dx());
+            if (fused_red) {
+                const int cb = d.cout[l - 1];
+                tail.kind |= DW_TAIL_BN_FINALIZE;
+                tail.red = fused_red; tail.red_parts = gemm_parts; tail.C = cb; tail.M = M; tail.accumulate = gr->acc_gb[l - 1] ? 1 : 0;
+                tail.dgamma = gr->dgamma[l - 1] ? gr->dgamma[l - 1] : b.tmp_gb; tail.dbeta = gr->dbeta[l - 1] ? gr->dbeta[l - 1] : b.tmp_gb + cmaxc;
+                tail.c1 = b.c12[l - 1]; tail.c2 = b.c12[l - 1] + cb;
+                fin_carried = true;
             }
-            dz = dz_prev;
-        } else if (x_needs) {
-            SA_CALL(papc_mlp_bwd_dx_f32(&dy, wts[l], M, cin, cout, gr->grad_x, nullptr, nullptr, st));
-        } else if (f_needs) {
-            SA_CALL(papc_fill_f32(gr->grad_feats, (int64_t)d.B * d.N * d.D, 0.f, st));
-            papc_scatter_dst sc;
-            memset(&sc, 0, sizeof(sc));
-            sc.grad_feats = gr->grad_feats; sc.idx = io->idx; sc.N = d.N; sc.S = d.S; sc.K = d.K; sc.D = d.D; sc.col0 = d.xyz_first ? 3 : 0;
-            SA_CALL(papc_mlp_bwd_dx_f32(&dy, wts[l], M, cin, cout, nullptr, &sc, nullptr, st));
-        }
+        }
+        const bool carries_fold = fold_pending && !(p.nostore && l == L - 1);
+        if (carries_fold) {
+            tail.kind |= DW_TAIL_MAX_FOLD;
+            tail.fpart = fold_job.fpart; tail.f_chunks = fold_job.f_chunks; tail.f_n = fold_job.f_n; tail.f_ld = fold_job.f_ld; tail.f_out = fold_job.f_out;
+        }
+        tail.n_units = dw_tail_bn_units(tail) + dw_tail_fold_units(tail);
+        SA_CALL(run_dw((tail.kind && carry) ? &tail : nullptr));
+        if (tail.kind && !carry) {
+            if (tail.kind & DW_TAIL_BN_FINALIZE)
+                SA_CALL(papc_bn_bwd_finalize_f32(tail.red, tail.red_parts, tail.M, tail.C, tail.dgamma, tail.dbeta, tail.c1, tail.c2, tail.accumulate, st));
+            if (tail.kind & DW_TAIL_MAX_FOLD) SA_CALL(mlp_bwd_dw_max_fold(&tail, st));
+        }
+        if (carries_fold) {
+            const int lm = L - 1, cm = d.cout[lm], ci = cin_of(p, lm);
+            SA_CALL(mlp_bwd_dw_max_finish(io->layer[lm].w, b.eq, s.cst[lm] + 2 * cm, b.c12[lm], M, ci, cm, b.dwmax_ws, gr->dw[lm], gr->acc_w[lm] ? 1 : 0, st));
+            fold_pending = false;
+        }
+        if (!dx_first) SA_CALL(run_dx());
     }
     if (n_jobs) SA_CALL(papc_reduce_partials_batch_f32(jobs, n_jobs, st));
     return PAPC_OK;
```

After: 22090. Within noise of the previous version (-1.0%).
